# NVorbis/NVorbis

Measured on AMD Instinct MI355X. Metric: decoded Vorbis frames/sec (44.1 kHz stereo long-block), higher is better.
Workload: dtype f32; 1 GPU; C2: 4096 stereo long-block (n=2048) frames, Floor1+Residue2+coupling, IMDCT+window+OLA; frames_per_gpu=4096, channels=2, block=2048, parallelism=frame-parallel x1, 3 HIP streams per GPU x 3 resident batches each

## Files before the change

include/nvorbis_hip.h:

```cpp
#ifndef NVORBIS_HIP_H
#define NVORBIS_HIP_H

#include <stddef.h>
#include <stdint.h>

#ifdef __cplusplus
extern "C" {
#endif

#define NVH_OK 0
#define NVH_ERR_INVALID_DATA (-1)
#define NVH_ERR_ARGUMENT (-2)
#define NVH_ERR_RUNTIME (-3)
#define NVH_ERR_NOMEM (-4)
#define NVH_ERR_NOT_VORBIS (-5)
#define NVH_ERR_DEVICE (-6)
#define NVH_ERR_UNSUPPORTED (-7)
#define NVH_ERR_NO_GPU (-8)

typedef struct nvh_ctx nvh_ctx;
typedef struct nvh_stream nvh_stream;
typedef struct nvh_batch nvh_batch;

#define NVH_PKT_EOS 1
// ... 46 lines not shown
int nvh_mdct_reverse(nvh_ctx *ctx, int n, int batch, float *d_buf, int64_t stride);

int nvh_mdct_tables(int n, float *a , float *b , float *c , uint16_t *bitrev );
int nvh_calc_window(int prev_block, int block, int next_block, float *out );
int nvh_calc_overlap(int prev_block, int block, int next_block, int *start, int *valid, int *total);


int nvh_stream_open(nvh_ctx *ctx, const uint8_t *id_pkt, int id_len, const uint8_t *comment_pkt, int comment_len,
                    const uint8_t *setup_pkt, int setup_len, nvh_stream **out);
void nvh_stream_close(nvh_stream *s);
int nvh_stream_bitrates(const nvh_stream *s, int *upper, int *nominal, int *lower);
int nvh_stream_info(const nvh_stream *s, int *channels, int *sample_rate, int *block0, int *block1);
int nvh_pinned_alloc(size_t bytes, void **out);
void nvh_pinned_free(void *p);
int nvh_stream_set_clip(nvh_stream *s, int on);
int nvh_stream_set_gpu_parse(nvh_stream *s, int on);
int nvh_stream_has_clipped(nvh_stream *s, int *clipped);
int nvh_stream_position(const nvh_stream *s, int64_t *position, int64_t *emitted, int *eos);

int nvh_stream_push_packet(nvh_stream *s, const uint8_t *data, int len, int64_t granule, int flags);
int nvh_stream_push_packets(nvh_stream *s, const uint8_t *bytes, const int64_t *offsets, const int64_t *granules,
                            const uint8_t *flags, int n, int max_packets, int *consumed);
int nvh_stream_position_state(const nvh_stream *s, int *has_position, int64_t *position);
int nvh_stream_set_position_state(nvh_stream *s, int has_position, int64_t position);
int nvh_stream_index_packets(const nvh_stream *s, const uint8_t *bytes, const int64_t *offsets, const int64_t *granules,
                             const uint8_t *flags, int n, int64_t *position_after, int64_t *emitted_after,
                             uint8_t *state_after, int64_t *total_emitted);
int nvh_stream_packet_sample_count(const nvh_stream *s, const uint8_t *pkt, int len, int is_resync, int *count);
int nvh_stream_reset(nvh_stream *s);
int nvh_stream_drop_pending(nvh_stream *s);
int nvh_stream_push_end(nvh_stream *s);
int nvh_stream_pending_geometry(const nvh_stream *s, int32_t *out, int cap_frames);
int nvh_stream_pending(const nvh_stream *s, int *frames, int64_t *pcm_samples_per_channel);
int nvh_stream_next_segment(nvh_stream *s, int align);
int nvh_stream_segment_window(nvh_stream *s, int64_t skip, int64_t take, int64_t pitch);
int nvh_stream_pending_segments(const nvh_stream *s, int64_t *index, int64_t *begin, int64_t *end, int cap, int *count);
int nvh_stream_synth_segments(const nvh_stream *s, int64_t *index, int64_t *begin, int64_t *end, int cap, int *count);
int nvh_stream_synth_segments_clipped(const nvh_stream *s, int32_t *clipped, int cap, int *count);
int nvh_stream_pending_slabs(const nvh_stream *s, uint8_t *buf, int64_t cap, int64_t *bytes, uint32_t *first_unit,
                             int cap_frames);
int nvh_stream_lattice_pool(const nvh_stream *s, uint32_t *out, int64_t cap_words, int64_t *words);
int nvh_stream_vq_pool(const nvh_stream *s, float *out, int64_t cap_floats, int64_t *floats);

typedef struct nvh_pcm_out {
  int32_t format;
  int32_t mix;
  int32_t planar;
  int32_t out_channels;
  const int32_t *map;
  int64_t extent;
} nvh_pcm_out;
int nvh_stream_synth_out(nvh_stream *s, const nvh_pcm_out *out, void *pcm_host, void *d_pcm, int64_t *written);
int nvh_stream_synth_begin_out(nvh_stream *s, const nvh_pcm_out *out, void *pcm_host, int64_t *expected);

int nvh_stream_synth(nvh_stream *s, float *pcm_host, float *d_pcm, int64_t capacity, int64_t *written);
int nvh_stream_synth_begin(nvh_stream *s, float *pcm_host, int64_t capacity, int64_t *expected);
int nvh_stream_synth_end(nvh_stream *s, int64_t *written);
#define NVH_PCM_F32 0
#define NVH_PCM_S16 1
int nvh_stream_synth_pcm(nvh_stream *s, int format, void *pcm_host, void *d_pcm, int64_t capacity, int64_t *written);
int nvh_stream_synth_begin_pcm(nvh_stream *s, int format, void *pcm_host, int64_t capacity, int64_t *expected);
int nvh_stream_synth_planar(nvh_stream *s, int format, void *pcm_host, void *d_pcm, int64_t plane_stride, int64_t *written);
int nvh_stream_synth_begin_planar(nvh_stream *s, int format, void *pcm_host, int64_t plane_stride, int64_t *expected);
#define NVH_MIX_NONE 0
#define NVH_MIX_MONO 1
int nvh_stream_synth_mix(nvh_stream *s, int format, int mix, void *pcm_host, void *d_pcm, int64_t capacity, int64_t *written);
int nvh_stream_synth_begin_mix(nvh_stream *s, int format, int mix, void *pcm_host, int64_t capacity, int64_t *expected);
int nvh_channel_map_wave(int channels, int32_t *map);
int nvh_stream_synth_map(nvh_stream *s, int format, const int32_t *map, int out_channels, void *pcm_host, void *d_pcm, int64_t capacity, int64_t *written);
int nvh_stream_synth_begin_map(nvh_stream *s, int format, const int32_t *map, int out_channels, void *pcm_host, int64_t capacity, int64_t *expected);
int nvh_stream_synth_planar_map(nvh_stream *s, int format, const int32_t *map, int out_channels, void *pcm_host, void *d_pcm, int64_t plane_stride, int64_t *written);
int nvh_stream_synth_begin_planar_map(nvh_stream *s, int format, const int32_t *map, int out_channels, void *pcm_host, int64_t plane_stride, int64_t *expected);
int nvh_stream_parse_errors(const nvh_stream *s, int32_t *codes, int64_t *samples_before, int cap, int *count);

int nvh_mode_decode(nvh_stream *s, const uint8_t *pkt, int len, float *d_block, int *decoded, int *block_size, int *start,
                    int *valid, int *total);

int nvh_batch_upload(nvh_stream *s, nvh_batch **out);
int nvh_batch_info(const nvh_batch *b, int *frames, int *chan_frames, int64_t *pcm_samples_per_channel,
                   int64_t *descriptor_bytes);
int nvh_batch_stats(const nvh_batch *b, int64_t *out8);
int nvh_batch_kernels(const nvh_batch *b, char *buf, int cap);
int nvh_stream_kernels(const nvh_stream *s, char *buf, int cap);
int nvh_batch_synth_out(nvh_batch *b, const nvh_pcm_out *out, void *d_pcm);
int nvh_batch_synth(nvh_batch *b, float *d_pcm, int64_t capacity);
int nvh_batch_synth_pcm(nvh_batch *b, int format, void *d_pcm, int64_t capacity);
int nvh_batch_synth_planar(nvh_batch *b, int format, void *d_pcm, int64_t plane_stride);
int nvh_batch_synth_mix(nvh_batch *b, int format, int mix, void *d_pcm, int64_t capacity);
int nvh_batch_synth_map(nvh_batch *b, int format, const int32_t *map, int out_channels, void *d_pcm, int64_t capacity);
int nvh_batch_synth_planar_map(nvh_batch *b, int format, const int32_t *map, int out_channels, void *d_pcm, int64_t plane_stride);
int nvh_batch_time(nvh_batch *b, float *d_pcm, int64_t capacity, int iters, float *total_ms, float *kernel_ms );
void nvh_batch_free(nvh_batch *b);

int nvh_ogg_demux(const uint8_t *bytes, size_t len, uint8_t *pkt_bytes, int64_t pkt_bytes_cap, int64_t *offsets,
                  int64_t *granules, uint8_t *flags, int pkt_cap, int *npackets, int64_t *total_bytes);
int nvh_ogg_demux_stream(const uint8_t *bytes, size_t len, int stream_index, uint8_t *pkt_bytes, int64_t pkt_bytes_cap,
                         int64_t *offsets, int64_t *granules, uint8_t *flags, int pkt_cap, int *npackets,
                         int64_t *total_bytes, int *nstreams);

int nvh_ogg_index_packets(const uint8_t *bytes, size_t len, int stream_index, uint8_t *pkt_bytes, int64_t pkt_bytes_cap,
                          int64_t *offsets, int64_t *granules, uint8_t *flags, int pkt_cap, int *npackets,
                          int64_t *total_bytes, int64_t *payload_bytes, int *nstreams);

int nvh_ogg_demux_forward(const uint8_t *bytes, size_t len, int stream_index, uint8_t *pkt_bytes, int64_t pkt_bytes_cap,
                          int64_t *offsets, int64_t *granules, uint8_t *flags, int pkt_cap, int *npackets,
                          int64_t *total_bytes, int *nstreams);

typedef struct nvh_ogg_index nvh_ogg_index;
int nvh_ogg_index_open(const uint8_t *bytes, size_t len, int stream_index, nvh_ogg_index **out);
void nvh_ogg_index_close(nvh_ogg_index *ix);
int nvh_ogg_index_info(const nvh_ogg_index *ix, int *npages, int *npackets, int *first_data_page, int64_t *max_granule,
                       int *has_all_pages);
int nvh_ogg_index_page(const nvh_ogg_index *ix, int page, int64_t *granule, int *flags, int *packet_count, int *first_packet);
int nvh_ogg_seek(const nvh_ogg_index *ix, const nvh_stream *s, int64_t granule_pos, int pre_roll, int64_t *packet_index,
                 int64_t *granule_out);

#define NVH_RESAMPLE_TILE 512
typedef struct nvh_resample_desc {
  int32_t in_rate, out_rate;
  int32_t rows;
  int32_t channels;
  int32_t format;
  int32_t reserved;
  int64_t length;
  int64_t src_length;
  int64_t src_row_stride, src_time_stride, src_chan_stride;
  int64_t dst_row_stride, dst_time_stride, dst_chan_stride;
} nvh_resample_desc;
int nvh_resample_plan(int in_rate, int out_rate, int *up, int *down, int *half, int64_t *tap_count);
int nvh_resample_taps(int in_rate, int out_rate, float *taps, int64_t cap, int64_t *count);
int nvh_resample_rows(nvh_ctx *ctx, const nvh_resample_desc *desc, const float *d_src, void *d_dst, const int64_t *origin,
                      const int64_t *start, const int64_t *valid, const int32_t *dst_row, int32_t *d_clipped);
int nvh_resample_route(const nvh_resample_desc *desc, int64_t *out);

#define NVH_MEL_HTK 0
#define NVH_MEL_SLANEY 1
#define NVH_MEL_NORM_NONE 0
#define NVH_MEL_NORM_SLANEY 1
#define NVH_MEL_POWER 0
#define NVH_MEL_LN 1
#define NVH_MEL_DB 2
#define NVH_MEL_FRAMES 4
typedef struct nvh_mel_desc {
  int32_t rate, n_fft, win_length, hop, n_mels;
  int32_t mel_scale, norm, scale;
  float floor;
  int32_t rows;
  int32_t channels;
  int32_t reserved;
  double f_min, f_max;
  int64_t frames;
  int64_t first;
  int64_t src_length;
  int64_t src_row_stride, src_time_stride, src_chan_stride;
  int64_t dst_row_stride, dst_chan_stride, dst_frame_stride, dst_band_stride;
} nvh_mel_desc;
int nvh_mel_plan(const nvh_mel_desc *desc, int64_t *twiddle_count, int64_t *window_count, int64_t *bank_count);
int nvh_mel_tables(const nvh_mel_desc *desc, float *twiddle, float *window, float *bank, int64_t twiddle_cap, int64_t window_cap,
                   int64_t bank_cap, int64_t *twiddle_count, int64_t *window_count, int64_t *bank_count);
int nvh_mel_rows(nvh_ctx *ctx, const nvh_mel_desc *desc, const float *d_src, float *d_dst, const int64_t *valid);

#define NVH_WIN_HANN 0
#define NVH_WIN_HANN_SYM 1
#define NVH_WIN_HAMMING 2
#define NVH_WIN_POVEY 3
#define NVH_WIN_RECT 4
// ... 88 lines not shown
```

nvorbis_amd/csrc/kernels_synth.hip:

```cpp
#include <hip/hip_runtime.h>

#include "imdct_wave.h"
#include "kernels_common.h"
#include "spectrum_dev.h"

#include <type_traits>

namespace {

#ifdef NVH_NO_SYNTH_PF
constexpr bool kSynthPF = false, kSynthPFEmit = false;
#else
constexpr bool kSynthPF = true, kSynthPFEmit = true;
#endif
#ifdef NVH_ABL_NO_XFORM
constexpr int kAblSkip = 3;
#else
constexpr int kAblSkip = 0;
#endif

template <int AUX = 0>
__device__ __forceinline__ void dma16(const uint4* __restrict__ gsrc, float* lds_chunk_base) {
  __builtin_amdgcn_global_load_lds((const __attribute__((address_space(1))) void*)gsrc,
                                   (__attribute__((address_space(3))) void*)lds_chunk_base, 16, 0, AUX);
// ... 160 lines not shown
        if (!mg1) {
#pragma unroll
          for (int m = 0; m < G / 2; ++m) couple1(a[2 * m], a[2 * m + 1]);
        } else {
#pragma unroll
          for (int m = 0; m < G / 2; ++m) couple1(a[2 * m + 1], a[2 * m]);
        }
      }
      float* p0 = spec + xb;
      float* p1 = spec + (unsigned)half + xb;
      if constexpr (FUSE && G == 8) {
        if (xb + 4 <= (unsigned)half) {
#pragma unroll
          for (int c = 0; c < 2; ++c) {
            if (F->md[c] == 1) {
              float m[4];
              floor_walk_fx<4>(F->seg[c], F->tab[c], F->s_db, (int)xb, m);
#pragma unroll
              for (int q = 0; q < 4; ++q) a[2 * q + c] = a[2 * q + c] * m[q];
            } else if (F->md[c] == 2) {
#pragma unroll
              for (int q = 0; q < 4; ++q) a[2 * q + c] = 0.0f;
            }
          }
          *reinterpret_cast<float4*>(p0) = make_float4(a[0], a[2], a[4 % G], a[6 % G]);
          *reinterpret_cast<float4*>(p1) = make_float4(a[1], a[3 % G], a[5 % G], a[7 % G]);
        }
      } else
      if (G == 8 && (xb & 3u) == 0 && xb + 4 <= (unsigned)half) {
        *reinterpret_cast<float4*>(p0) = make_float4(a[0], a[2], a[4 % G], a[6 % G]);
        *reinterpret_cast<float4*>(p1) = make_float4(a[1], a[3 % G], a[5 % G], a[7 % G]);
      } else {
#pragma unroll
        for (int m = 0; m < G / 2; ++m)
          if (xb + m < (unsigned)half) {
            p0[m] = a[2 * m];
            p1[m] = a[2 * m + 1];
          }
      }
    } else {
      const unsigned c = (rec.y >> 25) & 7u;
      const unsigned xb = xbase + i0;
      float* p = spec + c * (unsigned)half + xb;
      if constexpr (FUSE && G == 8) {
        if (xb + 8 <= (unsigned)half) {
          const bool c1 = c != 0;
          const int md = c1 ? F->md[1] : F->md[0];
          if (md == 1) {
            float m[8];
            floor_walk_fx<8>(c1 ? F->seg[1] : F->seg[0], c1 ? F->tab[1] : F->tab[0], F->s_db, (int)xb, m);
#pragma unroll
            for (int q = 0; q < 8; ++q) a[q % G] = a[q % G] * m[q];
          } else if (md == 2) {
#pragma unroll
            for (int q = 0; q < G; ++q) a[q] = 0.0f;
          }
          *reinterpret_cast<float4*>(p) = make_float4(a[0], a[1], a[2 % G], a[3 % G]);
          *reinterpret_cast<float4*>(p + 4) = make_float4(a[4 % G], a[5 % G], a[6 % G], a[7 % G]);
        } else if (xb + 4 <= (unsigned)half) {
          __builtin_trap();
        }
      } else
      if (G == 8 && (xb & 3u) == 0 && xb + 8 <= (unsigned)half) {
        *reinterpret_cast<float4*>(p) = make_float4(a[0], a[1], a[2 % G], a[3 % G]);
        *reinterpret_cast<float4*>(p + 4) = make_float4(a[4 % G], a[5 % G], a[6 % G], a[7 % G]);
      } else {
#pragma unroll
        for (int k = 0; k < G; ++k)
          if (xb + k < (unsigned)half) p[k] = a[k];
      }
    }
  }
}


struct WalkFrame {
  const float* slab;
  unsigned off_heads, off_rec, off_ent, nheads, lpc, lpc_magic, flags;
  float* spec;
  int half;
  FloorRef F;
};

template <int NT>
__device__ __forceinline__ void residue_walk_two(const WalkFrame (&W)[2], const uint32_t* __restrict__ s_lat, int tid) {
  constexpr int G = 8;
  const uint32_t* heads[2];
  const uint2* recs[2];
  const uint8_t* ent[2];
  unsigned total[2];
#pragma unroll
  for (int f = 0; f < 2; ++f) {
    heads[f] = reinterpret_cast<const uint32_t*>(W[f].slab + W[f].off_heads * 4);
    recs[f] = reinterpret_cast<const uint2*>(W[f].slab + W[f].off_rec * 4);
    ent[f] = reinterpret_cast<const uint8_t*>(W[f].slab + W[f].off_ent * 4);
    total[f] = W[f].nheads * W[f].lpc;
  }
  const unsigned tmax = total[0] > total[1] ? total[0] : total[1];
  for (unsigned idx = tid; idx < tmax; idx += NT) {
    bool act[2], more[2];
    unsigned o[2], xbase[2], i0[2];
    uint2 rec[2];
    float a[2][G];
#pragma unroll
    for (int f = 0; f < 2; ++f) {
      act[f] = idx < total[f];
      const unsigned ii = act[f] ? idx : 0u;
      const unsigned oq = W[f].lpc > 1 ? __umulhi(ii, W[f].lpc_magic) : ii;
      i0[f] = (ii - oq * W[f].lpc) * G;
      const unsigned hd = heads[f][oq];
      o[f] = hd & 0xFFFFu;
      xbase[f] = hd >> 16;
      rec[f] = recs[f][o[f]];
      more[f] = act[f];
#pragma unroll
      for (int k = 0; k < G; ++k) a[f][k] = 0.0f;
    }
#ifdef NVH_ABL_NO_CHAIN2
    more[0] = more[1] = false;
#endif
    while (more[0] | more[1]) {
      float v[2][G];
#pragma unroll
      for (int f = 0; f < 2; ++f) {
        const char* vb = reinterpret_cast<const char*>(s_lat) + ((rec[f].y & 0xFFFu) << 2);
        const uint8_t* db = ent[f] + ((rec[f].x & 0xFFFFu) << 1) + i0[f];
        const uint2 w = *reinterpret_cast<const uint2*>(db);
#pragma unroll
        for (int k = 0; k < 4; ++k) {
          v[f][k] = *reinterpret_cast<const float*>(vb + ((w.x >> (8 * k)) & 0xFFu));
          v[f][4 + k] = *reinterpret_cast<const float*>(vb + ((w.y >> (8 * k)) & 0xFFu));
        }
      }
#pragma unroll
      for (int f = 0; f < 2; ++f) {
        const uint32_t keep = more[f] ? 0xFFFFFFFFu : 0u;
#pragma unroll
        for (int k = 0; k < G; ++k) a[f][k] = a[f][k] + __uint_as_float(__float_as_uint(v[f][k]) & keep);
        more[f] = more[f] && (rec[f].y & 0x80000000u) != 0u;
        o[f] += more[f] ? 1u : 0u;
        rec[f] = recs[f][o[f]];
      }
    }
#pragma unroll
    for (int f = 0; f < 2; ++f) {
      if (!act[f]) continue;
      const unsigned xb = xbase[f] + (i0[f] >> 1);
      if (W[f].flags & NVH_SLAB_SWEEP_COUPLES) {
        if (!(W[f].flags & NVH_SLAB_MG1)) {
#pragma unroll
          for (int m = 0; m < G / 2; ++m) couple1(a[f][2 * m], a[f][2 * m + 1]);
        } else {
#pragma unroll
          for (int m = 0; m < G / 2; ++m) couple1(a[f][2 * m + 1], a[f][2 * m]);
        }
      }
      if (xb + 4 <= (unsigned)W[f].half) {
#pragma unroll
        for (int c = 0; c < 2; ++c) {
#ifdef NVH_ABL_NO_FLOOR2
          if (false) {
#else
          if (W[f].F.md[c] == 1) {
#endif
            float m[4];
            floor_walk_fx<4>(W[f].F.seg[c], W[f].F.tab[c], W[f].F.s_db, (int)xb, m);
#pragma unroll
            for (int q = 0; q < 4; ++q) a[f][2 * q + c] = a[f][2 * q + c] * m[q];
          } else if (W[f].F.md[c] == 2) {
#pragma unroll
            for (int q = 0; q < 4; ++q) a[f][2 * q + c] = 0.0f;
          }
        }
        *reinterpret_cast<float4*>(W[f].spec + xb) = make_float4(a[f][0], a[f][2], a[f][4], a[f][6]);
        *reinterpret_cast<float4*>(W[f].spec + (unsigned)W[f].half + xb) = make_float4(a[f][1], a[f][3], a[f][5], a[f][7]);
      }
    }
  }
}

template <int NT, bool DIG = false>
__device__ __forceinline__ void residue_walk_bins(const float* slab, unsigned off_heads, unsigned off_rec, unsigned off_ent,
                                                  unsigned off_bins, unsigned psz_magic, const uint32_t* __restrict__ s_lat,
                                                  float* spec, int half, unsigned rch, int tid, const float* __restrict__ vq = nullptr) {
  const uint32_t* heads = reinterpret_cast<const uint32_t*>(slab + off_heads * 4);
  const uint2* recs = reinterpret_cast<const uint2*>(slab + off_rec * 4);
  const uint16_t* ent = reinterpret_cast<const uint16_t*>(slab + off_ent * 4);
  const uint32_t* prm = reinterpret_cast<const uint32_t*>(slab + off_bins * 4);
  const unsigned rbegin = __builtin_amdgcn_readfirstlane(prm[0]), psz = __builtin_amdgcn_readfirstlane(prm[1]);
  const unsigned nparts = __builtin_amdgcn_readfirstlane(prm[2]), cover = __builtin_amdgcn_readfirstlane(prm[3]);
  const uint16_t* pchain = reinterpret_cast<const uint16_t*>(prm + 4);
  if (nparts == 0) return;
  const unsigned rch_magic = (unsigned)((0x100000000ull + rch - 1) / rch);
  auto base_of = [&](unsigned p) { return __umulhi(rbegin + p * psz, rch_magic); };
  const unsigned xfirst = base_of(0), xend = base_of(nparts - 1) + cover;
  for (unsigned X = xfirst + (unsigned)tid; X < xend; X += NT) {
    unsigned phi = __umulhi((X + 1) * rch - 1 - rbegin, psz_magic);
    if (phi >= nparts) phi = nparts - 1;
    unsigned cb = pchain[phi], ca = 0xFFFFu;
    if (X >= base_of(phi) + cover) cb = 0xFFFFu;
    if (phi >= 1 && X < base_of(phi - 1) + cover) ca = pchain[phi - 1];
    unsigned oa = 0, ob = 0, xa = 0, xbb = 0;
    uint2 ra = make_uint2(0u, 0u), rb = ra;
    bool va = ca != 0xFFFFu, vb = cb != 0xFFFFu;
    if (va) { const unsigned hd = heads[ca]; oa = hd & 0xFFFFu; xa = hd >> 16; ra = recs[oa]; }
    if (vb) { const unsigned hd = heads[cb]; ob = hd & 0xFFFFu; xbb = hd >> 16; rb = recs[ob]; }
    float a[NVH_SLAB_MAX_CH];
#pragma unroll
    for (int c = 0; c < NVH_SLAB_MAX_CH; ++c) a[c] = 0.0f;
    while (va || vb) {
      const bool take_a = va && (!vb || ((ra.y >> 28) & 7u) <= ((rb.y >> 28) & 7u));
      const uint2 rec = take_a ? ra : rb;
      const unsigned q0 = (X - (take_a ? xa : xbb)) * rch;
      if constexpr (DIG) {
        const char* vb = reinterpret_cast<const char*>(s_lat) + ((rec.y & 0xFFFu) << 2);
        const uint8_t* db = reinterpret_cast<const uint8_t*>(ent) + ((rec.x & 0xFFFFu) << 1);
#pragma unroll
        for (int c = 0; c < NVH_SLAB_MAX_CH; ++c) {
          if ((unsigned)c < rch) {
            const unsigned q = q0 + (unsigned)c;
            const bool in = q < psz;
            const float v = *reinterpret_cast<const float*>(vb + db[in ? q : 0u]);
            a[c] = a[c] + (in ? v : 0.0f);
          }
        }
      } else {
      const unsigned dims = (rec.y >> 20) & 31u, lv = (rec.y >> 12) & 0xFFu, dm16 = rec.x >> 16;
      const uint32_t* lat = s_lat + (rec.y & 0xFFFu);
      const uint16_t* eb = ent + (rec.x & 0xFFFFu);
      const unsigned lvm = lat[lv + 1];
#pragma unroll
      for (int c = 0; c < NVH_SLAB_MAX_CH; ++c) {
        if ((unsigned)c < rch) {
          const unsigned q = q0 + (unsigned)c;
          const bool in = q < psz;
          const unsigned qq = in ? q : 0u;
          const unsigned j = (qq * dm16) >> 16, comp = qq - j * dims;
          const unsigned e = eb[j];
          float v;
          if (lv == 0u) {
            v = table_value(vq, lat, dims, e, comp);
          } else {
            const unsigned pw = lat[lv + comp];
            const unsigned qv = comp ? __umulhi(e, pw) : e;
            const unsigned dgt = qv - __umul24(__umulhi(qv, lvm), lv);
            v = __uint_as_float(lat[dgt]);
// ... 961 lines not shown
  } else {
    bool kept = false;
    if constexpr (MAXCH > 2 && MODE >= 2) kept = xform && direct8;
    if constexpr (MAXCH > 2 && MODE >= 2) if (kept) {
      const float* X = spec + wv * half;
      float* scratch = smem + wv * (half + (n >> 4));
      switch (n) {
        case 256: imdct_keep_quarters<8>(X, scratch, Aa, Bb, Cc, TW, lane); break;
        case 512: imdct_keep_quarters<9>(X, scratch, Aa, Bb, Cc, TW, lane); break;
        case 1024: imdct_keep_quarters<10>(X, scratch, Aa, Bb, Cc, TW, lane); break;
        case 2048: imdct_keep_quarters<11>(X, scratch, Aa, Bb, Cc, TW, lane); break;
        case 4096: imdct_keep_quarters<12>(X, scratch, Aa, Bb, Cc, TW, lane); break;
        default: __builtin_trap();
      }
    }
    if (xform && !kept) {
      const float* X = spec + wv * half;
      float* out = planes + (long long)wv * A.block1;
      float* scratch = smem + wv * (half + (n >> 4));
      switch (n) {
        case 256: imdct_wave<8, false, true, true, true, false, true>(X, out, nullptr, scratch, Aa, Bb, Cc, TW, lane); break;
        case 512: imdct_wave<9, false, true, true, true, false, true>(X, out, nullptr, scratch, Aa, Bb, Cc, TW, lane); break;
        case 1024: imdct_wave<10, false, true, true, true, false, true>(X, out, nullptr, scratch, Aa, Bb, Cc, TW, lane); break;
        case 2048: imdct_wave<11, false, true, true, true, false, true>(X, out, nullptr, scratch, Aa, Bb, Cc, TW, lane); break;
        case 4096: imdct_wave<12, false, true, true, true, false, true>(X, out, nullptr, scratch, Aa, Bb, Cc, TW, lane); break;
        case 8192: {
          __syncthreads();
          float* own = spec + nch * half_max + wv * (half + (n >> 4));
          imdct_wave<13, false, true>(X, out, nullptr, own, Aa, Bb, Cc, TW, lane);
          break;
        }
        default: __builtin_trap();
      }
    }
  }
  if (!xform && wv < nch) {
    const float* X = spec + wv * half;
    float* out = planes + (long long)wv * A.block1;
    for (int i = lane * 4; i < half; i += 256) *reinterpret_cast<float4*>(out + i) = *reinterpret_cast<const float4*>(X + i);
    for (int i = lane * 4; i < (half >> 1); i += 256) *reinterpret_cast<float4*>(out + half + i) = make_float4(0.0f, 0.0f, 0.0f, 0.0f);
  }
  if (MAXCH > 2 && !xform) __syncthreads();
  if constexpr (MAXCH > 2 && MODE >= 2) {
    const unsigned ef = ef8;
    if (direct8) {
      __syncthreads();
      switch (nch) {
        case 1: synth_emit8_direct<NT, 1, PCM, LAYOUT>(A, smem, n, frame, tid, cm); break;
        case 2: synth_emit8_direct<NT, 2, PCM, LAYOUT>(A, smem, n, frame, tid, cm); break;
        case 3: synth_emit8_direct<NT, 3, PCM, LAYOUT>(A, smem, n, frame, tid, cm); break;
        case 4: synth_emit8_direct<NT, 4, PCM, LAYOUT>(A, smem, n, frame, tid, cm); break;
        case 5: synth_emit8_direct<NT, 5, PCM, LAYOUT>(A, smem, n, frame, tid, cm); break;
        case 6: synth_emit8_direct<NT, 6, PCM, LAYOUT>(A, smem, n, frame, tid, cm); break;
        case 7: synth_emit8_direct<NT, 7, PCM, LAYOUT>(A, smem, n, frame, tid, cm); break;
        case 8: synth_emit8_direct<NT, 8, PCM, LAYOUT>(A, smem, n, frame, tid, cm); break;
        default: __builtin_trap();
      }
    } else
    if (ef & (NVH_EMIT_SELF | NVH_EMIT_NEXT | NVH_EMIT_CARRY_OUT)) {
      __syncthreads();
      if ((ef & NVH_EMIT_CARRY_OUT) && A.carry_out) synth_carry_out8<NT>(A, planes, n, nch, exec_mask, A.frames[frame].window_off, tid);
      if (ef & (NVH_EMIT_SELF | NVH_EMIT_NEXT)) synth_emit8<NT, PCM, LAYOUT>(A, smem, n, nch, frame, ef, exec_mask, tid, cm);
    }
  }
  if constexpr (MAXCH > 2 && MODE < 2) {
    if (A.carry_out != nullptr && (A.frames[frame].emit_flags & NVH_EMIT_CARRY_OUT)) {
      __syncthreads();
      synth_carry_out8<NT>(A, planes, n, nch, exec_mask, A.frames[frame].window_off, tid);
    }
  }
  if constexpr (MAXCH <= 2 && MODE >= 1) {
    if (carry_out && !(emit_self || emit_next)) {
      __syncthreads();
      synth_carry_out<NT>(A, planes, n, nch, exec_mask, carry_window, tid);
    }
  }
  SY_T(5);
#ifdef NVH_DEBUG
  if (dbg && threadIdx.x == 0) dbg[(long long)f * 24 + 23] = wall_clock64();
#endif
#undef SY_T
}

template <int NT, int FPW, typename PCM = float, int LAYOUT = NVH_LAYOUT_INTERLEAVED>
__device__ __forceinline__ void synth_group_body(const NvhSynthArgs& A, float* smem NVH_DBG_PARAMS) {
  static_assert(NT / 64 >= 2 * FPW, "one wavefront per (frame, channel) in the transform");
  constexpr bool PLANAR = LAYOUT == NVH_LAYOUT_PLANAR, MONO = LAYOUT == NVH_LAYOUT_MONO;
  const int tid = threadIdx.x, wv = __builtin_amdgcn_readfirstlane(tid >> 6), lane = tid & 63;
  const int nch = A.channels;
  const int fa = A.f0 + (int)blockIdx.x * A.fstep;
#ifdef NVH_DEBUG
#define GR_T(k) do { if (dbg && tid == 0 && fa < A.nframes) dbg[(long long)fa * 24 + (k)] = clock64(); } while (0)
#else
#define GR_T(k) do { } while (0)
#endif
  GR_T(0);
  const int half_max = A.block1 >> 1, pad_max = A.block1 >> 4;
  float* s_db = smem;
  const uint32_t* s_lat = reinterpret_cast<const uint32_t*>(smem + 256);
  float* slab0 = smem + A.const_vecs * 4;
  const int slab_words = A.lds_vecs * 4;
  float* spec0 = slab0 + FPW * slab_words;
  const int region = nch * half_max;
  const int slice_words = half_max + pad_max;
  float* slice0 = smem + nch * half_max;
  const int walk_end = A.const_vecs * 4 + FPW * (slab_words + region), xform_end = nch * half_max + FPW * nch * slice_words;
  uint32_t* otab = reinterpret_cast<uint32_t*>(smem + (walk_end > xform_end ? walk_end : xform_end));
  typedef const __attribute__((address_space(4))) uint32_t* const_words;
  unsigned w0[FPW], w3[FPW];
#pragma unroll
  for (int k = 0; k < FPW; ++k) {
    w0[k] = 0u; w3[k] = 0u;
    if (fa + k < A.nframes) {
      const uint4* gslab = A.slabs + (long long)(fa + k) * A.stride_vecs;
      const_words gh = (const_words)(unsigned long long)gslab;
      w0[k] = gh[0]; w3[k] = gh[3];
      if (tid < A.cap_vecs) dma16<kSlabAux>(gslab + tid, slab0 + k * slab_words + wv * 256);
    }
  }
  for (int c0 = wv * 64; c0 < A.const_vecs; c0 += NT)
    if (c0 + lane < A.const_vecs) dma16(A.consts + c0 + lane, smem + c0 * 4);
  {
    const float4 z = make_float4(0.0f, 0.0f, 0.0f, 0.0f);
#pragma unroll
    for (int k = 0; k < FPW; ++k) {
      float4* sp = reinterpret_cast<float4*>(spec0 + k * region);
      for (int i = tid; i < (nch * half_max) >> 2; i += NT) sp[i] = z;
    }
  }
  int nn[FPW];
  bool any = false;
#pragma unroll
  for (int k = 0; k < FPW; ++k) {
    nn[k] = (int)(w0[k] & 0xFFFFu);
    any = any || nn[k] != 0;
    const unsigned vecs = w3[k] >> 16;
    if ((int)vecs > A.cap_vecs) __builtin_trap();
    if (vecs > (unsigned)NT) {
      const uint4* gslab = A.slabs + (long long)(fa + k) * A.stride_vecs;
      for (unsigned c0 = NT + wv * 64; c0 < vecs; c0 += NT)
        if (c0 + lane < vecs) dma16<kSlabAux>(gslab + c0 + lane, slab0 + k * slab_words + c0 * 4);
    }
  }
  if (A.prefetch_prev && wv == NT / 64 - 1 && fa >= FPW) {
    const int lines = (A.cap_vecs < 256 ? A.cap_vecs : 256) >> 3;
#pragma unroll
    for (int k = 0; k < FPW; ++k)
      if (lane < lines) {
        const volatile unsigned* pp = reinterpret_cast<const volatile unsigned*>(A.slabs + (long long)(fa - FPW + k) * A.stride_vecs) + lane * 32;
        (void)*pp;
      }
  }
  __syncthreads();
  if (!any) return;
  GR_T(1);

  auto hdr = [&](int k, int i) { return __builtin_amdgcn_readfirstlane(reinterpret_cast<const uint32_t*>(slab0 + k * slab_words)[i]); };
  {
    bool together = false;
    if constexpr (FPW == 2) {
      WalkFrame W[2];
      together = A.walk_two != 0;
#pragma unroll
      for (int k = 0; k < 2; ++k) {
        const unsigned w1 = hdr(k, 1), w2 = hdr(k, 2), w4 = hdr(k, 4), flags = w0[k] >> 24, rgeom = (w4 >> 16) & 0xFFu;
        W[k].slab = slab0 + k * slab_words;
        W[k].nheads = w1 & 0xFFFFu; W[k].off_heads = w2 & 0xFFFFu; W[k].off_rec = w2 >> 16; W[k].off_ent = w3[k] & 0xFFFFu;
        W[k].lpc = w4 & 0xFFFFu; W[k].lpc_magic = hdr(k, 5); W[k].flags = flags;
        W[k].spec = spec0 + k * region; W[k].half = nn[k] >> 1;
        together = together && nn[k] != 0 && (flags & NVH_SLAB_FUSE_FLOOR) && !(flags & NVH_SLAB_FLOOR_FAULT) &&
                   rgeom == (2u | NVH_SLAB_RGEOM_DIGITS | (2u << 4)) && (w4 >> 24) == 8u && W[k].nheads * W[k].lpc != 0u;
        const uint32_t* s_chan = reinterpret_cast<const uint32_t*>(W[k].slab) + 8;
        const unsigned c0w = __builtin_amdgcn_readfirstlane(s_chan[0]), c1w = __builtin_amdgcn_readfirstlane(s_chan[1]);
        const unsigned cw[2] = {c0w, c1w};
#pragma unroll
        for (int c = 0; c < 2; ++c) {
          const unsigned ns = (cw[c] >> 8) & 0xFFu, oseg = cw[c] >> 16;
          W[k].F.seg[c] = reinterpret_cast<const uint4*>(W[k].slab + oseg * 4);
          W[k].F.tab[c] = reinterpret_cast<const uint8_t*>(W[k].slab + (oseg + ns) * 4);
          W[k].F.md[c] = (int)(cw[c] & 0xFFu);
        }
        W[k].F.s_db = s_db;
      }
      if (together) residue_walk_two<NT>(W, s_lat, tid);
      if (together) { GR_T(2); GR_T(3); }
    }
    if (!together)
#pragma unroll
    for (int k = 0; k < FPW; ++k) {
      if (nn[k] != 0)
        synth_frame_spectrum<NT, 2, false>(A, s_db, s_lat, slab0 + k * slab_words, spec0 + k * region, w0[k], hdr(k, 1), hdr(k, 2),
                                           w3[k], hdr(k, 4), hdr(k, 5), hdr(k, 7), tid);
      if (k < 2) GR_T(2 + k);
    }
  }

  const bool emit = A.pcm != nullptr;
  bool self_k[FPW], next_k[FPW], cout_k[FPW], done_k[FPW];
  bool self_carry = false;
  int gprev[FPW], gnext[FPW], gstart[FPW], gvalid[FPW];
#pragma unroll
  for (int k = 0; k < FPW; ++k) {
    const unsigned flags = w0[k] >> 24, xm = (w0[k] >> 16) & 0xFFu;
    self_k[k] = emit && nn[k] != 0 && (flags & NVH_SLAB_EMIT_SELF);
    next_k[k] = emit && nn[k] != 0 && (flags & NVH_SLAB_EMIT_NEXT);
    done_k[k] = emit && nn[k] != 0 && (xm & NVH_SLABX_DONE);
    cout_k[k] = A.carry_out != nullptr && nn[k] != 0 && (xm & NVH_SLABX_CARRY_OUT);
    if (k == 0) self_carry = self_k[0] && (xm & NVH_SLABX_SELF_CARRY);
    const unsigned geo = (self_k[k] || next_k[k] || done_k[k]) ? hdr(k, 13) : 0u;
    gprev[k] = (int)(geo & 0xFFu) << 6; gnext[k] = (int)((geo >> 8) & 0xFFu) << 6;
    gstart[k] = (int)((geo >> 16) & 0xFFu) << 6; gvalid[k] = (int)(geo >> 24) << 6;
  }
  bool act[FPW + 1];
  act[0] = self_k[0] && !self_carry;
#pragma unroll
  for (int j = 1; j < FPW; ++j) act[j] = next_k[j - 1] && self_k[j] && nn[j] == gnext[j - 1];
  act[FPW] = next_k[FPW - 1];
  int mov[FPW + 1];
  mov[0] = nn[0] < gprev[0] ? nn[0] : gprev[0];
#pragma unroll
  for (int j = 1; j <= FPW; ++j) mov[j] = nn[j - 1] < gnext[j - 1] ? nn[j - 1] : gnext[j - 1];
  int r1len[FPW], r2len[FPW];
#pragma unroll
  for (int k = 0; k < FPW; ++k) {
    const int mk = nn[k] < gprev[k] ? nn[k] : gprev[k];
    r1len[k] = done_k[k] ? (nn[k] >> 1) - gstart[k] - (mk >> 1) : 0;
    r2len[k] = done_k[k] ? gvalid[k] - (nn[k] >> 1) : 0;
    if (r1len[k] < 0 || r2len[k] < 0 || r1len[k] > (nn[k] >> 2) || r2len[k] > (nn[k] >> 2)) __builtin_trap();
  }
  const int S0 = (int)(slice0 - smem), SK = nch * slice_words;
  if (tid <= FPW) {
    const int j = tid, kb = j == 0 ? 0 : j - 1;
    const uint32_t* H = reinterpret_cast<const uint32_t*>(slab0 + kb * slab_words);
    const int n = (int)(H[0] & 0xFFFFu);
    const unsigned geo = H[13];
    uint4 r0, r1;
    if (j == 0) {
      const int pn = (int)(geo & 0xFFu) << 6, m = n < pn ? n : pn, start = (int)((geo >> 16) & 0xFFu) << 6;
// ... 51 lines not shown
    bool wrA = true, wrB = true, keep = false;
#pragma unroll
    for (int kk = 0; kk < FPW; ++kk)
      if (kk == k) {
        n = nn[kk]; mw0 = w0[kk];
        const bool a_here = kk == 0 ? self_k[0] : act[kk], b_here = kk == FPW - 1 ? next_k[FPW - 1] : act[kk + 1];
        wrA = !a_here || cout_k[kk] || !done_k[kk];
        wrB = !b_here || cout_k[kk] || !done_k[kk];
        keep = a_here || b_here || done_k[kk];
      }
    const unsigned exec_mask = (mw0 >> 16) & 0xFFu, flags = mw0 >> 24;
    const int half = n >> 1;
    const int sl = (flags & NVH_SLAB_MDCT_SLOT) ? 1 : 0;
    const float* X = spec0 + k * region + c * half;
    float* slice = slice0 + (k * nch + c) * slice_words;
    float* plane = A.work + ((long long)(fa + k) * nch + c) * A.block1;
    const bool mine = tw && c < nch && n != 0;
    if (mine && !((exec_mask >> c) & 1u)) {
      for (int i = lane * 4; i < half; i += 256) *reinterpret_cast<float4*>(plane + i) = *reinterpret_cast<const float4*>(X + i);
      for (int i = lane * 4; i < (half >> 1); i += 256) *reinterpret_cast<float4*>(plane + half + i) = make_float4(0.0f, 0.0f, 0.0f, 0.0f);
    }
    if (mine && ((exec_mask >> c) & 1u)) {
      float4 ca[2] = {make_float4(0.f, 0.f, 0.f, 0.f), make_float4(0.f, 0.f, 0.f, 0.f)}, cb[2] = {ca[0], ca[0]};
      auto sink = [&](int slot, int, float4 v) {
        if (slot == 0) ca[0] = v; else if (slot == 2) cb[0] = v; else if (slot == 4) ca[1] = v; else if (slot == 6) cb[1] = v;
      };
      const float* Aa = A.mdct_a[sl];
      const float* Bb = A.mdct_b[sl];
      const float* Cc = A.mdct_c[sl];
      const float* TW = A.mdct_tw[sl];
      switch (n) {
        case 256: imdct_wave_sink<8, false, decltype(sink), true, true, false, kSynthPFEmit, true>(X, nullptr, slice, Aa, Bb, Cc, TW, lane, sink, nullptr, kAblSkip); break;
        case 512: imdct_wave_sink<9, false, decltype(sink), true, true, false, kSynthPFEmit, true>(X, nullptr, slice, Aa, Bb, Cc, TW, lane, sink, nullptr, kAblSkip); break;
        case 1024: imdct_wave_sink<10, false, decltype(sink), true, true, false, kSynthPFEmit, true>(X, nullptr, slice, Aa, Bb, Cc, TW, lane, sink, nullptr, kAblSkip); break;
        case 2048: imdct_wave_sink<11, false, decltype(sink), true, true, false, kSynthPFEmit, true>(X, nullptr, slice, Aa, Bb, Cc, TW, lane, sink, nullptr, kAblSkip); break;
        default: __builtin_trap();
      }
      if (lane < (n >> 5)) {
        const int i8a = lane, i8b = (n >> 4) - 1 - lane;
        if (wrA) {
          *reinterpret_cast<float4*>(plane + 4 * i8a) = ca[0];
          *reinterpret_cast<float4*>(plane + 4 * i8b) = ca[1];
        }
        if (wrB) {
          *reinterpret_cast<float4*>(plane + half + 4 * i8a) = cb[0];
          *reinterpret_cast<float4*>(plane + half + 4 * i8b) = cb[1];
        }
        if (keep) {
          float* own = slice;
          *reinterpret_cast<float4*>(own + 4 * i8a) = ca[0];
          *reinterpret_cast<float4*>(own + 4 * i8b) = ca[1];
          *reinterpret_cast<float4*>(own + (half >> 1) + 4 * i8a) = cb[0];
          *reinterpret_cast<float4*>(own + (half >> 1) + 4 * i8b) = cb[1];
        }
      }
    } else {
      lds_barrier();
    }
  }
  GR_T(5);
  __syncthreads();
  GR_T(6);

#pragma unroll
  for (int k = 0; k < FPW; ++k)
    if (cout_k[k])
      synth_carry_out<NT>(A, A.work + (long long)(fa + k) * nch * A.block1, nn[k], nch, (w0[k] >> 16) & 0xFFu, cwin[k], tid);
  if (self_carry)
    synth_self_carry<NT, PCM, LAYOUT>(A, slice0, nn[0], nch, __builtin_amdgcn_readfirstlane(otab[0]), __builtin_amdgcn_readfirstlane(otab[2]), tid, fa, slice_words);

  int cnt[FPW + 2];
  cnt[0] = 0;
#pragma unroll
  for (int j = 0; j <= FPW; ++j) cnt[j + 1] = cnt[j] + (act[j] ? (mov[j] >> 4) : 0);
  int clipped = 0;
  for (int t = tid; t < cnt[FPW + 1]; t += NT) {
    int j = 0;
#pragma unroll
    for (int jj = 1; jj <= FPW; ++jj) j += (int)(t >= cnt[jj]);
    int g = t;
#pragma unroll
    for (int jj = 1; jj <= FPW; ++jj) g = j == jj ? t - cnt[jj] : g;
    const uint4 r0 = reinterpret_cast<const uint4*>(otab)[2 * j], r1 = reinterpret_cast<const uint4*>(otab)[2 * j + 1];
    const int n = (int)r0.w, half = n >> 1, i0 = 4 * g;
    const int cbit = 1 << j;
    const float* __restrict__ w = A.windows + r0.x;
    const float* __restrict__ wp = A.windows + r0.y;
    const float4 wf = *reinterpret_cast<const float4*>(w + i0);
    const float4 wm = *reinterpret_cast<const float4*>(w + (half - 4 - i0));
    const float4 pf = *reinterpret_cast<const float4*>(wp + i0);
    const float4 pm = *reinterpret_cast<const float4*>(wp + (half - 4 - i0));
    float fwd[8], mir[8];
#pragma unroll
    for (int c = 0; c < 2; ++c) {
      if (c < nch) {
        const float4 a = *reinterpret_cast<const float4*>(smem + r1.x + c * r1.y + i0);
        const float4 b = *reinterpret_cast<const float4*>(smem + r1.z + c * r1.w + i0);
        float4 v = make_float4(a.x * wf.x, a.y * wf.y, a.z * wf.z, a.w * wf.w);
        const float4 tt = make_float4(b.x * pf.x, b.y * pf.y, b.z * pf.z, b.w * pf.w);
        v.x = v.x + tt.x; v.y = v.y + tt.y; v.z = v.z + tt.z; v.w = v.w + tt.w;
        float4 u = make_float4(-a.w * wm.x, -a.z * wm.y, -a.y * wm.z, -a.x * wm.w);
        const float4 r = make_float4(b.w * pm.x, b.z * pm.y, b.y * pm.z, b.x * pm.w);
        u.x = u.x + r.x; u.y = u.y + r.y; u.z = u.z + r.z; u.w = u.w + r.w;
        if (!MONO && A.clip) {
          v.x = clip_value(v.x, &clipped, cbit); v.y = clip_value(v.y, &clipped, cbit);
          v.z = clip_value(v.z, &clipped, cbit); v.w = clip_value(v.w, &clipped, cbit);
          u.x = clip_value(u.x, &clipped, cbit); u.y = clip_value(u.y, &clipped, cbit);
          u.z = clip_value(u.z, &clipped, cbit); u.w = clip_value(u.w, &clipped, cbit);
        }
        if constexpr (PLANAR) {
          pcm_store_plane(reinterpret_cast<PCM*>(A.pcm) + (long long)r0.z + (long long)c * A.plane_stride, g, (n >> 3) - 1 - g, v, u);
        } else {
          fwd[c] = v.x; fwd[2 + c] = v.y; fwd[4 + c] = v.z; fwd[6 + c] = v.w;
            mir[c] = u.x; mir[2 + c] = u.y; mir[4 + c] = u.z; mir[6 + c] = u.w;
        }
      }
    }
    PCM* out = reinterpret_cast<PCM*>(A.pcm) + (long long)r0.z * (PLANAR || MONO ? 1 : nch);
    if constexpr (PLANAR) {
    } else if constexpr (MONO) {
      pcm_store_plane(out, g, (n >> 3) - 1 - g, mono_mix2(fwd, nch, A.clip, &clipped, cbit), mono_mix2(mir, nch, A.clip, &clipped, cbit));
    } else if (nch == 2) {
      pcm4_t<PCM>* of = reinterpret_cast<pcm4_t<PCM>*>(out) + 2 * (long long)g;
      pcm4_t<PCM>* om = reinterpret_cast<pcm4_t<PCM>*>(out) + 2 * (long long)((n >> 3) - 1 - g);
      if constexpr (std::is_same<PCM, int16_t>::value) {
        pcm_store4x2(of, fwd);
        pcm_store4x2(om, mir);
      } else {
        pcm_store4(of, fwd[0], fwd[1], fwd[2], fwd[3]);
        pcm_store4(of + 1, fwd[4], fwd[5], fwd[6], fwd[7]);
        pcm_store4(om, mir[0], mir[1], mir[2], mir[3]);
        pcm_store4(om + 1, mir[4], mir[5], mir[6], mir[7]);
      }
    } else {
      pcm_store4(reinterpret_cast<pcm4_t<PCM>*>(out) + g, fwd[0], fwd[2], fwd[4], fwd[6]);
      pcm_store4(reinterpret_cast<pcm4_t<PCM>*>(out) + ((n >> 3) - 1 - g), mir[0], mir[2], mir[4], mir[6]);
    }
  }
  int fcnt[FPW + 1];
  fcnt[0] = 0;
#pragma unroll
  for (int k = 0; k < FPW; ++k) fcnt[k + 1] = fcnt[k] + ((r1len[k] + r2len[k]) >> 2);
  for (int t = tid; t < fcnt[FPW]; t += NT) {
    int k = 0;
#pragma unroll
    for (int kk = 1; kk < FPW; ++kk) k += (int)(t >= fcnt[kk]);
    int g = t;
#pragma unroll
    for (int kk = 1; kk < FPW; ++kk) g = k == kk ? t - fcnt[kk] : g;
    const uint4 r0 = reinterpret_cast<const uint4*>(otab)[2 * (FPW + 1 + k)], r1 = reinterpret_cast<const uint4*>(otab)[2 * (FPW + 1 + k) + 1];
    const int n = (int)r0.z, q1 = (int)(r1.y >> 2);
    const bool second = g >= q1;
    const int cbit = 1 << k;
    const int idx0 = second ? (n >> 1) + 4 * (g - q1) : (int)r1.x + 4 * g;
    const float4 wv4 = *reinterpret_cast<const float4*>(A.windows + r0.x + idx0);
    const int src = second ? (n >> 2) + (idx0 - (n >> 1)) : (n >> 1) - 4 - idx0;
    float o[8];
#pragma unroll
    for (int c = 0; c < 2; ++c) {
      if (c < nch) {
        const float4 x = *reinterpret_cast<const float4*>(smem + r0.w + c * slice_words + src);
        float4 v = second ? make_float4(x.x * wv4.x, x.y * wv4.y, x.z * wv4.z, x.w * wv4.w)
                          : make_float4(-x.w * wv4.x, -x.z * wv4.y, -x.y * wv4.z, -x.x * wv4.w);
        if (!MONO && A.clip) {
          v.x = clip_value(v.x, &clipped, cbit); v.y = clip_value(v.y, &clipped, cbit);
          v.z = clip_value(v.z, &clipped, cbit); v.w = clip_value(v.w, &clipped, cbit);
        }
        if constexpr (PLANAR)
          pcm_store4(reinterpret_cast<pcm4_t<PCM>*>(reinterpret_cast<PCM*>(A.pcm) + ((long long)r0.y + (idx0 - (int)r1.w)) +
                                                    (long long)c * A.plane_stride), v.x, v.y, v.z, v.w);
        else {
          o[c] = v.x; o[2 + c] = v.y; o[4 + c] = v.z; o[6 + c] = v.w;
        }
      }
    }
    PCM* out = reinterpret_cast<PCM*>(A.pcm) + ((long long)r0.y + (idx0 - (int)r1.w)) * (PLANAR || MONO ? 1 : nch);
    if constexpr (PLANAR) {
    } else if constexpr (MONO) {
      const float4 m = mono_mix2(o, nch, A.clip, &clipped, cbit);
      pcm_store4(reinterpret_cast<pcm4_t<PCM>*>(out), m.x, m.y, m.z, m.w);
    } else if (nch == 2) {
      if constexpr (std::is_same<PCM, int16_t>::value) {
        pcm_store4x2(reinterpret_cast<pcm4_t<PCM>*>(out), o);
      } else {
        pcm_store4(reinterpret_cast<float4*>(out), o[0], o[1], o[2], o[3]);
        pcm_store4(reinterpret_cast<float4*>(out) + 1, o[4], o[5], o[6], o[7]);
      }
    } else {
      pcm_store4(reinterpret_cast<pcm4_t<PCM>*>(out), o[0], o[2], o[4], o[6]);
    }
  }
  if (A.clip && emit) report_clipped<FPW + 1>(clipped, A.clipped_flag, fa);
  GR_T(7);
#undef GR_T
}

#ifndef NVH_SYNTH_NT
#define NVH_SYNTH_NT SP_THREADS
#define NVH_SYNTH_WPE 8, 8
#endif
extern "C" __global__ void __launch_bounds__(NVH_SYNTH_NT) __attribute__((amdgpu_waves_per_eu(NVH_SYNTH_WPE)))
k_synth(NvhSynthArgs A NVH_DBG_PARAMS) {
  extern __shared__ __attribute__((aligned(16))) float smem[];
  synth_body<NVH_SYNTH_NT, 2>(A, smem NVH_DBG_ARGS);
}

extern "C" __global__ void __launch_bounds__(NVH_SYNTH_NT) __attribute__((amdgpu_waves_per_eu(NVH_SYNTH_WPE)))
k_synth_tail(NvhSynthArgs A NVH_DBG_PARAMS) {
  extern __shared__ __attribute__((aligned(16))) float smem[];
  synth_body<NVH_SYNTH_NT, 2, 1>(A, smem NVH_DBG_ARGS);
}

#define NVH_SYNTH_EMIT(PCM, LAYOUT, SFX)                                                                                   \
  extern "C" __global__ void __launch_bounds__(NVH_SYNTH_NT) __attribute__((amdgpu_waves_per_eu(NVH_SYNTH_WPE)))           \
  k_synth_emit##SFX(NvhSynthArgs A NVH_DBG_PARAMS) {                                                                       \
    extern __shared__ __attribute__((aligned(16))) float smem[];                                                           \
    synth_body<NVH_SYNTH_NT, 2, 2, false, PCM, LAYOUT>(A, smem NVH_DBG_ARGS);                                              \
  }
NVH_FOR_PCM_TWINS(NVH_SYNTH_EMIT)

// ... 46 lines not shown
```

nvorbis_amd/csrc/nvh_api.hip:

```cpp
#include "nvh_internal.h"

#include <bitset>

thread_local int g_last_hip_error = 0;

const NvhToggles& nvh_toggles() {
  static const NvhToggles t = [] {
    auto on = [](const char* k) { return std::getenv(k) != nullptr; };
    auto num = [](const char* k) { const char* v = std::getenv(k); return v ? std::atoi(v) : 0; };
    NvhToggles x{};
    x.no_compact = on("NVH_NO_COMPACT");
    x.no_fused_imdct = on("NVH_NO_FUSED_IMDCT");
    x.no_gen8 = on("NVH_NO_GEN8");
    x.unfused = on("NVH_UNFUSED");
    x.no_pair = on("NVH_NO_PAIR");
    x.no_slab = on("NVH_NO_SLAB");
    x.uncached_planes = on("NVH_UNCACHED_PLANES");
    x.poison_planes = on("NVH_POISON_PLANES");
    x.no_ola_sym = on("NVH_NO_OLA_SYM");
    x.no_emit = on("NVH_NO_EMIT");
    x.emit8 = on("NVH_EMIT8");
    x.no_emit8 = on("NVH_NO_EMIT8");
    x.no_prefetch = on("NVH_NO_PREFETCH");
    x.no_walk_two = on("NVH_NO_WALK_TWO");
    x.fpw = std::getenv("NVH_FPW") ? num("NVH_FPW") : 2;
    if (x.fpw != 1 && x.fpw != 2 && x.fpw != 4) x.fpw = 2;
    x.copy_upload = on("NVH_COPY_UPLOAD");
    x.xcd_map = on("NVH_XCD_MAP");
    x.emit_always = on("NVH_EMIT_ALWAYS");
    x.debug_occ = on("NVH_DEBUG_OCC");
    x.gpu_parse_default = on("NVH_GPU_PARSE");
    x.lds_pad = num("NVH_LDS_PAD");
    x.ola_threads = num("NVH_OLA_THREADS");
    x.parse_lanes = num("NVH_PARSE_LANES");
    x.parse_waves = num("NVH_PARSE_WAVES");
    x.no_parse_uni = on("NVH_NO_PARSE_UNI");
    x.no_parse_sub = on("NVH_NO_PARSE_SUB");
    x.parse_cur = std::getenv("NVH_PARSE_CUR") ? num("NVH_PARSE_CUR") : -1;
    if (x.parse_cur > 2) x.parse_cur = 2;
    x.no_sleep_wait = on("NVH_NO_SLEEP_WAIT");
    x.no_parse_sort = on("NVH_NO_PARSE_SORT");
    x.ola_segs = num("NVH_OLA_SEGS");
    x.zero_chunk_kib = num("NVH_ZERO_CHUNK_KIB");
    x.phase_mask = std::getenv("NVH_DEBUG_SPECTRUM_MASK") ? num("NVH_DEBUG_SPECTRUM_MASK") : 15;
    return x;
  }();
  return t;
}

#ifdef NVH_DEBUG
void* g_dbg_buf = nullptr;
extern "C" void nvh_debug_set_buffer(void* d_buf) { g_dbg_buf = d_buf; }
#endif

static int ensure_device(int device) {
  int count = 0;
  hipError_t e = hipGetDeviceCount(&count);
  if (e != hipSuccess || count <= 0) {
    g_last_hip_error = (int)e;
    return NVH_ERR_NO_GPU;
  }
  if (device < 0 || device >= count) return NVH_ERR_ARGUMENT;
  HIP_TRY(hipSetDevice(device));
  return NVH_OK;
}

#ifndef NVH_SRC_HASH
#define NVH_SRC_HASH "unknown"
#endif
extern "C" const char* nvh_version(void) { return "nvorbis_hip 0.3 (gfx950) nvh-src-hash=" NVH_SRC_HASH; }
extern "C" int nvh_last_hip_error(void) { return g_last_hip_error; }
extern "C" int nvh_device_count(void) {
  int count = 0;
  if (hipGetDeviceCount(&count) != hipSuccess) return 0;
  return count;
}

extern "C" int nvh_ctx_create(int device, nvh_ctx** out) {
  return nvh_guard([&]() -> int {
    if (!out) return NVH_ERR_ARGUMENT;
    *out = nullptr;
    int rc = ensure_device(device);
    if (rc != NVH_OK) return rc;
    nvh_ctx* c = new (std::nothrow) nvh_ctx();
    if (!c) return NVH_ERR_NOMEM;
    c->device = device;
    c->hpool.host = true;
    hipError_t e = hipStreamCreateWithFlags(&c->stream, hipStreamNonBlocking);
    if (e != hipSuccess) {
      g_last_hip_error = (int)e;
      delete c;
      return NVH_ERR_DEVICE;
    }
    c->own_stream = true;
    *out = c;
    return NVH_OK;
  });
}

extern "C" void nvh_ctx_destroy(nvh_ctx* c) {
  nvh_guard_void([&] {
    if (!c) return;
    (void)hipSetDevice(c->device);
    for (auto& kv : c->mdct_cache) kv.second.free_tables();
    for (auto& kv : c->resample_cache) (void)hipFree(kv.second.taps);
    c->resample_rows.release();
    for (auto& kv : c->mel_cache) kv.second.free_tables();
// ... 830 lines not shown
    return F.replay_error;
  });
}

extern "C" int nvh_stream_parse_errors(const nvh_stream* s, int32_t* codes, int64_t* samples_before, int cap, int* count) {
  return nvh_guard([&]() -> int {
    if (!s || !count || cap < 0 || (cap > 0 && (!codes || !samples_before))) return NVH_ERR_ARGUMENT;
    const int n = s->replay_error != NVH_OK ? (int)s->replay_errors.size() : 0;
    *count = n;
    for (int i = 0; i < n && i < cap; i++) {
      codes[i] = s->replay_errors[(size_t)i].first;
      samples_before[i] = s->replay_errors[(size_t)i].second;
    }
    return NVH_OK;
  });
}

extern "C" int nvh_batch_upload(nvh_stream* s, nvh_batch** out) {
  return nvh_guard([&]() -> int {
    if (!s || !out) return NVH_ERR_ARGUMENT;
    *out = nullptr;
    if (!s->ctx) return NVH_ERR_NO_GPU;
    HIP_TRY(hipSetDevice(s->ctx->device));
    std::unique_ptr<nvh_batch> b(new (std::nothrow) nvh_batch());
    if (b && s && s->ctx) {
      b->blob.pool = b->work.pool = b->carry_in.pool = b->slabs.pool = b->dev_copy.pool = b->slab3.pool = b->gap_dev.pool = &s->ctx->pool;
      b->work.uncached = nvh_toggles().uncached_planes;
      b->h_blob.host = b->gap_host.host = true;
      b->h_blob.pool = b->gap_host.pool = &s->ctx->hpool;
    }
    if (!b) return NVH_ERR_NOMEM;
    size_t plane = (size_t)s->setup.channels * (size_t)s->setup.block1 * sizeof(float);
    int rc = b->carry_in.reserve(plane);
    if (rc != NVH_OK) return rc;
    HIP_TRY(hipMemcpyAsync(b->carry_in.p, s->carry[s->carry_cur].p, plane, hipMemcpyDeviceToDevice, s->ctx->stream));
    b->has_carry_in = true;
    s->replay_error = NVH_OK;
    rc = batch_upload(s, b.get());
    if (rc != NVH_OK) return rc;
    if (s->replay_error != NVH_OK) return s->replay_error;
    *out = b.release();
    return NVH_OK;
  });
}

extern "C" int nvh_batch_info(const nvh_batch* b, int* frames, int* chan_frames, int64_t* pcm_samples,
                              int64_t* descriptor_bytes) {
  return nvh_guard([&]() -> int {
    if (!b) return NVH_ERR_ARGUMENT;
    if (frames) *frames = b->nframes;
    if (chan_frames) *chan_frames = b->chan_frames;
    if (pcm_samples) *pcm_samples = b->pcm_samples;
    if (descriptor_bytes) *descriptor_bytes = b->descriptor_bytes;
    return NVH_OK;
  });
}

extern "C" int nvh_batch_stats(const nvh_batch* b, int64_t* out8) {
  return nvh_guard([&]() -> int {
    if (!b || !out8) return NVH_ERR_ARGUMENT;
    for (int i = 0; i < 8; i++) out8[i] = b->stats[i];
    return NVH_OK;
  });
}

extern "C" int nvh_batch_kernels(const nvh_batch* b, char* buf, int cap) {
  return nvh_guard([&]() -> int {
    if (!b || !buf || cap <= 0) return NVH_ERR_ARGUMENT;
    std::string t;
    for (int k = 0; k < 4; k++) {
      if (k) t += ",";
      t += b->slot_name[k];
    }
    if ((int)t.size() + 1 > cap) return NVH_ERR_ARGUMENT;
    std::memcpy(buf, t.c_str(), t.size() + 1);
    return NVH_OK;
  });
}

extern "C" int nvh_stream_kernels(const nvh_stream* s, char* buf, int cap) {
  return nvh_batch_kernels(s ? &s->scratch : nullptr, buf, cap);
}

static int batch_out(nvh_batch* b, const nvh_pcm_out* d, void* d_pcm, NamedForm form = kDescriptor) {
  return nvh_guard([&]() -> int {
    nvh_stream* s = b ? b->s : nullptr;
    PcmOut out;
    const int rc = resolve_out(s, b, d, form, false, nullptr, d_pcm, nullptr, &out);
    if (rc != NVH_OK) return rc;
    HIP_TRY(hipSetDevice(s->ctx->device));
    return batch_launch(b, (const float*)b->carry_in.p, (float*)s->carry[s->carry_cur].p, d_pcm, false, nullptr, nullptr, out);
  });
}

extern "C" int nvh_batch_synth_out(nvh_batch* b, const nvh_pcm_out* out, void* d_pcm) { return batch_out(b, out, d_pcm); }

extern "C" int nvh_batch_synth(nvh_batch* b, float* d_pcm, int64_t capacity) {
  const nvh_pcm_out d{NVH_PCM_F32, NVH_MIX_NONE, 0, 0, nullptr, capacity};
  return nvh_batch_synth_out(b, &d, d_pcm);
}

extern "C" int nvh_batch_synth_pcm(nvh_batch* b, int format, void* d_pcm, int64_t capacity) {
  const nvh_pcm_out d{format, NVH_MIX_NONE, 0, 0, nullptr, capacity};
  return nvh_batch_synth_out(b, &d, d_pcm);
}

extern "C" int nvh_batch_synth_mix(nvh_batch* b, int format, int mix, void* d_pcm, int64_t capacity) {
  const nvh_pcm_out d{format, mix, 0, 0, nullptr, capacity};
  return nvh_batch_synth_out(b, &d, d_pcm);
}

extern "C" int nvh_batch_synth_planar(nvh_batch* b, int format, void* d_pcm, int64_t plane_stride) {
  const nvh_pcm_out d{format, NVH_MIX_NONE, 1, 0, nullptr, plane_stride};
  return nvh_batch_synth_out(b, &d, d_pcm);
}

extern "C" int nvh_batch_synth_map(nvh_batch* b, int format, const int32_t* map, int out_channels, void* d_pcm, int64_t capacity) {
  const nvh_pcm_out d{format, NVH_MIX_NONE, 0, out_channels, map, capacity};
  return batch_out(b, &d, d_pcm, kNamedMap);
}

extern "C" int nvh_batch_synth_planar_map(nvh_batch* b, int format, const int32_t* map, int out_channels, void* d_pcm,
                                          int64_t plane_stride) {
  const nvh_pcm_out d{format, NVH_MIX_NONE, 1, out_channels, map, plane_stride};
  return batch_out(b, &d, d_pcm, kNamedMap);
}

extern "C" int nvh_batch_time(nvh_batch* b, float* d_pcm, int64_t capacity, int iters, float* total_ms,
                              float* kernel_ms) {
  return nvh_guard([&]() -> int {
    if (!b || !b->s || iters <= 0) return NVH_ERR_ARGUMENT;
    nvh_stream* s = b->s;
    if (capacity < b->pcm_samples * s->setup.channels) return NVH_ERR_ARGUMENT;
    HIP_TRY(hipSetDevice(s->ctx->device));
    hipStream_t st = s->ctx->stream;
    float km[4] = {0, 0, 0, 0};
    if (kernel_ms) {
      std::vector<ScopedEvent> evs((size_t)iters * 5);
      std::vector<hipEvent_t> raw((size_t)iters * 5);
      for (size_t k = 0; k < evs.size(); k++) {
        int rc = evs[k].create();
        if (rc != NVH_OK) return rc;
        raw[k] = evs[k].e;
      }
      for (int i = 0; i < iters; i++) {
        int rc = batch_launch(b, (const float*)b->carry_in.p, (float*)s->carry[s->carry_cur].p, d_pcm, true, km, &raw[(size_t)i * 5]);
        if (rc != NVH_OK) return rc;
      }
      HIP_TRY(hipEventSynchronize(raw.back()));
      for (int i = 0; i < iters; i++)
        for (int k = 0; k < 4; k++) {
          float ms = 0;
          HIP_TRY(hipEventElapsedTime(&ms, raw[(size_t)i * 5 + k], raw[(size_t)i * 5 + k + 1]));
          km[k] += ms;
        }
      for (int k = 0; k < 4; k++) kernel_ms[k] = km[k] / (float)iters;
    }
    if (total_ms) {
      ScopedEvent e0, e1;
      int rc = e0.create();
      if (rc == NVH_OK) rc = e1.create();
      if (rc != NVH_OK) return rc;
      HIP_TRY(hipEventRecord(e0.e, st));
      for (int i = 0; i < iters; i++) {
        rc = batch_launch(b, (const float*)b->carry_in.p, (float*)s->carry[s->carry_cur].p, d_pcm, false, nullptr);
        if (rc != NVH_OK) return rc;
// ... 220 lines not shown
```

nvorbis_amd/csrc/nvh_format.h:

```cpp
#pragma once
#include <stdint.h>

#define NVH_MAX_POSTS 64
#define NVH_LINK_NONE 0x7FFF
#define NVH_MAX_STAGES 8
#define NVH_MAX_CLASSES 64
#define NVH_ENTRY_SKIP 0xFFFFu


struct NvhDevBook {
  uint32_t tab_off;
  uint32_t entries;
  uint32_t dim;
  uint32_t dim_magic;
  uint32_t lat_values;
  uint32_t lat_magic;
  uint32_t lat_off;
  uint32_t dim_magic16;
};

struct NvhDevFloor1 {
  int32_t x_count;
  int32_t multiplier;
  int32_t range;
// ... 38 lines not shown
  int32_t pair_path;
  uint32_t hp_magic;
  int32_t alias_b1;
  int32_t pad[2];
};

struct NvhDevMapping {
  int32_t coupling_steps;
  uint32_t coupling_off;
};


struct NvhResOp {
  uint32_t ent_off;
  uint16_t partition;
  uint8_t channel;
  uint8_t book;
};

struct NvhResPass {
  int32_t residue;
  uint32_t op_begin[NVH_MAX_STAGES + 1];
};

struct NvhChan {
  uint8_t exec;
  uint8_t floor;
  uint8_t post_count;
  uint8_t ov_exec;
  uint32_t data_off;
  float amp;
};

struct NvhFrame {
  int32_t n;
  int32_t mapping;
  uint32_t window_off;
  int32_t mdct_slot;
  int32_t start, valid, total;
  int32_t emit_start;
  int32_t emit_count;
  int32_t ov_frame;
  int32_t ov_src;
  int32_t ov_len;
  int64_t out_pos;
  uint32_t chan_off;
  uint32_t pass_begin, pass_end;
  uint32_t op_begin, op_count;
  uint32_t ent_begin, ent_count;
  int32_t ov_n;
  uint32_t ov_window_off;
  uint32_t exec_mask;
  uint32_t ov_exec_mask;
  uint32_t emit_flags;
};

#define NVH_EMIT_SELF 1u
#define NVH_EMIT_NEXT 2u
#define NVH_EMIT_DONE 4u
#define NVH_EMIT_SELF_CARRY 8u
#define NVH_EMIT_CARRY_OUT 16u

#define NVH_SLAB_REC(ent_off, dm16, lat_off, lat_values, dim, channel, stage, more)                                              \
  ((uint32_t)(ent_off) | ((uint32_t)(dm16) << 16)),                                                                               \
      ((uint32_t)(lat_off) | ((uint32_t)(lat_values) << 12) | ((uint32_t)(dim) << 20) | ((uint32_t)(channel) << 25) |             \
       ((uint32_t)(stage) << 28) | ((more) ? 0x80000000u : 0u))
#define NVH_SLAB_MAX_LAT_OFF 0xFFFu
#define NVH_SLAB_RGEOM_DIGITS 8u
#define NVH_SLAB_MAX_DIGIT 63u
#define NVH_SLAB_SWEEP_COUPLES 1u
#define NVH_SLAB_MG1 2u
#define NVH_SLAB_COUPLE_PASS 4u
#define NVH_SLAB_FLOOR_FAULT 8u
#define NVH_SLAB_MDCT_SLOT 16u
#define NVH_SLAB_FUSE_FLOOR 32u
#define NVH_SLAB_EMIT_SELF 64u
#define NVH_SLAB_EMIT_NEXT 128u
#define NVH_SLABX_SELF_CARRY 0x40u
#define NVH_SLABX_CARRY_OUT 0x80u
#define NVH_SLABX_DONE 0x20u
#define NVH_SLAB_GEO(prev_n, next_n, start, valid) \
  ((uint32_t)((prev_n) >> 6) | ((uint32_t)((next_n) >> 6) << 8) | ((uint32_t)((start) >> 6) << 16) | ((uint32_t)((valid) >> 6) << 24))
#define NVH_SLAB_HDR_VECS 4
#define NVH_SLAB_MAX_CH 8
#define NVH_SLAB_MAX_COUPLE 4
struct NvhSlabHdr {
  uint16_t n;
  uint8_t exec_mask;
  uint8_t flags;
  uint16_t nheads, nrec;
  uint16_t off_heads, off_rec;
  uint16_t off_ent;
  uint16_t vecs;
  uint16_t lpc;
  uint8_t rgeom;
  uint8_t group;
  uint32_t lpc_magic;
  uint32_t frame;
  uint32_t coupling;
  uint32_t chan[NVH_SLAB_MAX_CH];
};
```

nvorbis_amd/csrc/nvh_internal.h:

```cpp
#pragma once
#include <time.h>
#include <hip/hip_runtime.h>

#include <algorithm>
#include <cstdio>
#include <cstdlib>
#include <cstring>
#include <initializer_list>
#include <iterator>
#include <map>
#include <memory>
#include <new>
#include <string>
#include <tuple>
#include <vector>

#include "../../include/nvorbis_hip.h"
#include "host_ogg.h"
#include "host_parse.h"
#include "host_setup.h"
#include "host_slab.h"
#include "kernels_common.h"
#include "nvh_parse_format.h"
#include "cep_dev.h"
// ... 67 lines not shown

template <typename PCM, int LAYOUT>
__global__ void k_ola_compact(NvhDevSetup S, NvhDevBatch Bt, const float* work, const float* carry, PCM* pcm, int clip,
                              int* clipped_flag, float* carry_out, int last_decoded, int nosym, const int* list, int emitted,
                              pcm_stride_t<LAYOUT> plane_stride);
template <typename PCM, int LAYOUT>
__global__ void k_ola_emit(NvhDevSetup S, NvhDevBatch Bt, const float* work, const float* carry, PCM* pcm, int clip, int* clipped_flag,
                           pcm_stride_t<LAYOUT> plane_stride);
template <typename PCM, int LAYOUT>
__global__ void k_ola_emit_seq(NvhDevSetup S, NvhDevBatch Bt, float* work, const float* carry, PCM* pcm, int clip, int* clipped_flag,
                               pcm_stride_t<LAYOUT> plane_stride);
#define NVH_OLA_DECL(PCM, LAYOUT, SFX)                                                                                               \
  extern template __global__ void k_ola_compact<PCM, LAYOUT>(NvhDevSetup, NvhDevBatch, const float*, const float*, PCM*, int, int*,  \
                                                             float*, int, int, const int*, int, pcm_stride_t<LAYOUT>);               \
  extern template __global__ void k_ola_emit<PCM, LAYOUT>(NvhDevSetup, NvhDevBatch, const float*, const float*, PCM*, int, int*,     \
                                                          pcm_stride_t<LAYOUT>);                                                     \
  extern template __global__ void k_ola_emit_seq<PCM, LAYOUT>(NvhDevSetup, NvhDevBatch, float*, const float*, PCM*, int, int*,       \
                                                              pcm_stride_t<LAYOUT>);
NVH_FOR_PCM_TWINS(NVH_OLA_DECL)
NVH_FOR_PCM_MAP_TWINS(NVH_OLA_DECL)

template <typename PCM>
__global__ void k_resample_rows(NvhResampleArgs A);
extern template __global__ void k_resample_rows<float>(NvhResampleArgs);
extern template __global__ void k_resample_rows<int16_t>(NvhResampleArgs);

template <bool STAGED, bool FRONT>
__global__ void k_mel_rows(NvhMelArgs A);
extern template __global__ void k_mel_rows<true, false>(NvhMelArgs);
extern template __global__ void k_mel_rows<false, false>(NvhMelArgs);
extern template __global__ void k_mel_rows<true, true>(NvhMelArgs);
extern template __global__ void k_mel_rows<false, true>(NvhMelArgs);

template <bool RESIDENT>
__global__ void k_fnorm_rows(NvhFnormArgs A);
extern template __global__ void k_fnorm_rows<true>(NvhFnormArgs);
extern template __global__ void k_fnorm_rows<false>(NvhFnormArgs);

template <bool STAGED>
__global__ void k_cep_rows(NvhCepArgs A);
extern template __global__ void k_cep_rows<true>(NvhCepArgs);
extern template __global__ void k_cep_rows<false>(NvhCepArgs);

extern thread_local int g_last_hip_error;

#define HIP_TRY(expr)                        \
  do {                                       \
    hipError_t e_ = (expr);                  \
    if (e_ != hipSuccess) {                  \
      g_last_hip_error = (int)e_;            \
      return NVH_ERR_DEVICE;                 \
    }                                        \
  } while (0)

template <class F>
static inline int nvh_guard(F&& body) noexcept {
  try {
    return body();
  } catch (const std::bad_alloc&) {
    return NVH_ERR_NOMEM;
  } catch (...) {
    return NVH_ERR_RUNTIME;
  }
}
template <class F>
static inline void nvh_guard_void(F&& body) noexcept {
  try {
    body();
  } catch (...) {
  }
}

struct NvhToggles {
  bool no_compact, no_fused_imdct, no_gen8, unfused, no_pair, debug_occ, gpu_parse_default;
  bool no_ola_sym;
  bool emit8;
  bool no_emit8;
  bool no_emit;
  bool emit_always;
  bool xcd_map;
  bool copy_upload;
  int fpw;
  bool no_walk_two;
  bool no_prefetch;
  bool uncached_planes;
  bool poison_planes;
  bool no_slab;
  int lds_pad, ola_threads, parse_lanes, parse_waves;
  bool no_sleep_wait;
  bool no_parse_sort;
  int parse_cur;
  bool no_parse_sub;
  bool no_parse_uni;
  int ola_segs;
  int zero_chunk_kib;
  int phase_mask;
};
const NvhToggles& nvh_toggles();
#ifdef NVH_DEBUG
extern void* g_dbg_buf;
#define NVH_DBG_LAUNCH , (long long*)g_dbg_buf, nvh_toggles().phase_mask
#else
#define NVH_DBG_LAUNCH
#endif

struct BufPool {
  bool host = false;
  std::multimap<size_t, void*> free_;
  size_t bytes_ = 0;
  void raw_free(void* p) const { (void)(host ? hipHostFree(p) : hipFree(p)); }
  static constexpr size_t kKeepBytes = (size_t)2 << 30;
  static size_t size_class(size_t bytes) {
    size_t v = bytes < 4096 ? 4096 : bytes;
    size_t p = 1;
    while ((p << 1) <= v) p <<= 1;
    size_t step = p >> 2;
    return (v + step - 1) / step * step;
  }
  void* take(size_t cls) {
    auto it = free_.find(cls);
    if (it == free_.end()) return nullptr;
    void* p = it->second;
    free_.erase(it);
    bytes_ -= cls;
    return p;
  }
  void give(void* p, size_t cls) {
    if (bytes_ + cls > kKeepBytes) {
      raw_free(p);
      return;
    }
    free_.emplace(cls, p);
    bytes_ += cls;
  }
  void clear() {
    for (auto& kv : free_) raw_free(kv.second);
    free_.clear();
    bytes_ = 0;
  }
};

struct DevBuf {
  void* p = nullptr;
  size_t cap = 0;
  BufPool* pool = nullptr;
  bool host = false;
  bool uncached = false;
  ~DevBuf() { release(); }
  void release() {
    if (!p) return;
    if (pool && !uncached) pool->give(p, cap);
    else (void)(host ? hipHostFree(p) : hipFree(p));
    p = nullptr;
    cap = 0;
  }
  int reserve(size_t bytes) {
    if (bytes <= cap) return NVH_OK;
    release();
    const size_t want = BufPool::size_class(bytes + 256);
    if (pool && !uncached) p = pool->take(want);
    if (!p) {
      if (host) HIP_TRY(hipHostMalloc(&p, want, hipHostMallocDefault));
      else if (uncached) HIP_TRY(hipExtMallocWithFlags(&p, want, hipDeviceMallocUncached));
      else HIP_TRY(hipMalloc(&p, want));
    }
    cap = want;
    return NVH_OK;
  }
};

template <class T>
static inline int upload_table(T** dst, const std::vector<T>& src) {
  void* p = nullptr;
  HIP_TRY(hipMalloc(&p, src.empty() ? 4 : src.size() * sizeof(T)));
  const hipError_t e = src.empty() ? hipSuccess : hipMemcpy(p, src.data(), src.size() * sizeof(T), hipMemcpyHostToDevice);
  if (e != hipSuccess) {
    (void)hipFree(p);
    g_last_hip_error = (int)e;
    return NVH_ERR_DEVICE;
  }
  *dst = static_cast<T*>(p);
// ... 67 lines not shown
  BufPool pool;
  BufPool hpool;
  std::map<std::string, std::shared_ptr<SharedSetup>> setup_cache;
  bool big_lds_attr_set = false;
  bool group_lds_attr_set = false;
  bool synth_lds_attr_set = false;
  bool parse_lds_attr_set = false;
  int parse_lanes = 0;
  std::map<std::pair<int, int>, ResampleDev> resample_cache;
  std::map<MelKey, MelDev> mel_cache;
  std::map<CepKey, CepDev> cep_cache;
  bool resample_lds_attr_set = false, mel_lds_attr_set = false, fnorm_lds_attr_set = false, cep_lds_attr_set = false;
  RowBlock resample_rows, mel_rows, fnorm_rows, cep_rows;
};

inline int RowBlock::begin(nvh_ctx* c, size_t bytes, void** image) {
  if (!copied) HIP_TRY(hipEventCreateWithFlags(&copied, hipEventDisableTiming));
  else HIP_TRY(hipEventSynchronize(copied));
  host.host = true;
  host.pool = &c->hpool;
  dev.pool = &c->pool;
  int rc = host.reserve(bytes);
  if (rc == NVH_OK) rc = dev.reserve(bytes);
  if (rc == NVH_OK) *image = host.p;
  return rc;
}

inline int RowBlock::send(nvh_ctx* c, size_t bytes, const void** d_block) {
  HIP_TRY(hipMemcpyAsync(dev.p, host.p, bytes, hipMemcpyHostToDevice, c->stream));
  HIP_TRY(hipEventRecord(copied, c->stream));
  *d_block = dev.p;
  return NVH_OK;
}

static inline int lds_opt_in(bool& done, int bytes, std::initializer_list<const void*> kernels) {
  if (done) return NVH_OK;
  for (const void* k : kernels) HIP_TRY(hipFuncSetAttribute(k, hipFuncAttributeMaxDynamicSharedMemorySize, bytes));
  done = true;
  return NVH_OK;
}

inline hipError_t nvh_wait_stream(const nvh_ctx* c, hipStream_t st) {
  if (!c || c->parse_lanes <= 0 || nvh_toggles().no_sleep_wait) return hipStreamSynchronize(st);
  for (;;) {
    const hipError_t e = hipStreamQuery(st);
    if (e != hipErrorNotReady) return e;
    struct timespec ts = {0, 50 * 1000};
    nanosleep(&ts, nullptr);
  }
}

struct nvh_batch {
  nvh_stream* s = nullptr;
  DevBuf blob;
  DevBuf h_blob;
  DevBuf slabs;
  DevBuf work;
  DevBuf carry_in;
  NvhDevBatch dev{};
  int nframes = 0, chan_frames = 0;
  int64_t pcm_samples = 0;
  int64_t descriptor_bytes = 0;
  int64_t stats[8] = {0, 0, 0, 0, 0, 0, 0, 0};
  bool sequential_ola = false;
  int last_decoded = -1;
  const char* slot_name[4] = {"-", "-", "-", "-"};
  std::string slot_name_buf[4];
  bool links_ok = false;
  int max_ops = 0, max_ent = 0, max_pass = 0;
  int max_vecs = 0;
  bool block_only = false;
  bool descriptors_only = false;
  bool has_carry_in = false;
  DevBuf dev_copy;
  bool dev_copy_valid = false;
  DevBuf slab3;
  int slab_stride_vecs = 0;
  int slab_cap_vecs = 0;
  bool slabs_ready = false;
  bool slab_host = false;
  const uint4* d_slabs = nullptr;
  int emit_frames = 0;
  bool emit_planar_ok = true;
  int fpw = 1;
  bool ola_all = false;
  int ola_count = 0;
  const int* d_ola_list = nullptr;
  std::vector<nvh::FrameBatch::Gap> gaps;
  DevBuf gap_dev, gap_host;
  std::vector<nvh::FrameBatch::Gap> row_chunks;
  std::vector<nvh::FrameBatch::Segment> segments;
  bool want_seg_flags = false;
  bool seg_table = false;
  DevBuf seg_dev, seg_image;
  int* seg_table_dev() const { return seg_table ? (int*)((uint8_t*)seg_dev.p + 8) : nullptr; }
  int* seg_flags_dev() const { return seg_table ? seg_table_dev() + nframes : nullptr; }
};

struct ReplayLog {
  enum { kPacket = 0, kEnd = 1, kPosition = 2, kSegment = 3, kWindow = 4 };
  struct Event { int kind; int64_t off, len, granule; int flags; };
  std::vector<uint8_t> bytes;
  std::vector<Event> events;
  void clear() { bytes.clear(); events.clear(); }
};

#define NVH_INTERNAL_REPLAY 1000

struct nvh_stream {
  nvh_ctx* ctx = nullptr;
  std::shared_ptr<SharedSetup> shared;
  nvh::Setup& setup;
  DevBuf& arena;
  NvhDevSetup& dev;
  bool& fast_spectrum;
  bool& has_floor0;
  std::unique_ptr<nvh::StreamParser> parser;
  nvh::FrameBatch pending;
  nvh::SlabBatch slab_build;
  DevBuf carry[2];
  int carry_cur = 0;
  DevBuf flags;
  int* seg_table_set = nullptr;
  DevBuf pcm;
  DevBuf h_pcm;
  int clip = 1;
  int has_clipped = 0;
  bool gpu_parse = false;
  DevBuf carry_exec;
  nvh_batch scratch;
  ReplayLog replay;
  std::unique_ptr<nvh::StreamParser> replay_start;
  int replay_error = NVH_OK;
  std::vector<nvh::FrameBatch::Segment> synth_segments;
  std::vector<int32_t> synth_clipped;
  DevBuf h_seg_flags[2];
  std::vector<std::pair<int, int64_t>> replay_errors;
  struct Flight {
    bool on = false;
    hipEvent_t kernels = nullptr, done = nullptr;
    int64_t need = 0;
    int replay_error = NVH_OK;
    std::vector<std::pair<int, int64_t>> replay_errors;
    std::vector<nvh::FrameBatch::Segment> segments;
    int seg_flag_words = 0;
  };
  hipStream_t copy_stream = nullptr;
  DevBuf pcm2[2];
  DevBuf h_flags2;
  Flight flight[2];
  int flight_next = 0, flight_first = 0;
  ~nvh_stream() {
    for (Flight& f : flight) {
      if (f.kernels) (void)hipEventDestroy(f.kernels);
      if (f.done) (void)hipEventDestroy(f.done);
    }
    if (copy_stream) (void)hipStreamDestroy(copy_stream);
  }

  nvh_stream(nvh_ctx* c, std::shared_ptr<SharedSetup> sh)
      : ctx(c), shared(std::move(sh)), setup(shared->setup), arena(shared->arena), dev(shared->dev),
        fast_spectrum(shared->fast_spectrum), has_floor0(shared->has_floor0) {
    BufPool* pool = c ? &c->pool : nullptr;
    carry[0].pool = carry[1].pool = flags.pool = pcm.pool = carry_exec.pool = pcm2[0].pool = pcm2[1].pool = pool;
    h_flags2.host = true;
    h_flags2.pool = c ? &c->hpool : nullptr;
// ... 74 lines not shown
```

nvorbis_amd/csrc/nvh_launch.hip:

```cpp
#include <array>
#include <chrono>

#include "nvh_internal.h"

static int collect_parse_result(nvh_stream* s, nvh_batch* b, const NvhParseResult* d_res);
static bool slab_shape_ok(const nvh_batch* b);
static bool slab_size_ok(const nvh_batch* b);
static void assign_emission(nvh_stream* s, nvh_batch* b, nvh::FrameBatch& P, int fpw, std::vector<int>& ola_list);
static int batch_upload_frames(nvh_stream* s, nvh_batch* b);

void replay_note(nvh_stream* s, int kind, const uint8_t* data, int len, int64_t granule, int flags) {
  if (!s->gpu_parse) return;
  if (s->replay.events.empty()) s->replay_start.reset(new nvh::StreamParser(*s->parser));
  ReplayLog::Event e{kind, (int64_t)s->replay.bytes.size(), (int64_t)len, granule, flags};
  if (kind == ReplayLog::kPacket && len > 0) s->replay.bytes.insert(s->replay.bytes.end(), data, data + len);
  s->replay.events.push_back(e);
}

void replay_note_window(nvh_stream* s, int64_t skip, int64_t take, int64_t pitch) {
  if (!s->gpu_parse) return;
  if (s->replay.events.empty()) s->replay_start.reset(new nvh::StreamParser(*s->parser));
  s->replay.events.push_back(ReplayLog::Event{ReplayLog::kWindow, skip, take, pitch, 0});
}

// ... 201 lines not shown
                         (int)nf, (NvhFrame*)(base + o_fr), (NvhChan*)(base + o_ch), (NvhResPass*)(base + o_ps), (NvhResOp*)(base + o_op),
                         (uint16_t*)(base + o_lk), (uint16_t*)(base + o_en), (uint16_t*)(base + o_po), (int*)(base + o_sc),
                         (NvhParseResult*)(base + o_rs), lanes, (int)sub_words, 0, (uint4*)b->slab3.p,
                         sorted_parse ? (const int*)(base + o_od) : (const int*)nullptr, (uint32_t*)(base + o_ho) NVH_DBG_LAUNCH);
      pkt_words = -1;
    }
    hipLaunchKernelGGL(cur ? k_parse_slab_c : uni ? k_parse_slab_u : slab_mode ? (in_lds ? k_parse_slab : k_parse_slab_g) : (in_lds ? k_parse : k_parse_g),
                       dim3(pblocks), dim3(64 * kParseWaves), parse_lds, st, T,
                       (const uint8_t*)(base + o_pk), (const NvhPacketRef*)(base + o_rf),
                       (int)nf, (NvhFrame*)(base + o_fr), (NvhChan*)(base + o_ch), (NvhResPass*)(base + o_ps), (NvhResOp*)(base + o_op),
                       (uint16_t*)(base + o_lk), (uint16_t*)(base + o_en), (uint16_t*)(base + o_po), (int*)(base + o_sc),
                       (NvhParseResult*)(base + o_rs), lanes, scratch_words, pkt_words, slab_mode ? (uint4*)b->slab3.p : (uint4*)nullptr,
                       sorted_parse ? (const int*)(base + o_od) : (const int*)nullptr, (uint32_t*)(base + o_ho) NVH_DBG_LAUNCH);
    if (cur) {
      constexpr int kTailWaves = 4;
      const size_t tail_lds = ((size_t)T.meta_words + 3 + (size_t)kTailWaves * (NVH_SP_FLOOR_SCRATCH_WORDS + 1) + 8) * sizeof(uint32_t);
      hipLaunchKernelGGL(k_parse_slab_t, dim3((unsigned)((nf + kTailWaves - 1) / kTailWaves)), dim3(64 * kTailWaves), tail_lds, st, T,
                         (const uint8_t*)(base + o_pk), (const NvhPacketRef*)(base + o_rf),
                         (int)nf, (NvhFrame*)(base + o_fr), (NvhChan*)(base + o_ch), (NvhResPass*)(base + o_ps), (NvhResOp*)(base + o_op),
                         (uint16_t*)(base + o_lk), (uint16_t*)(base + o_en), (uint16_t*)(base + o_po), (int*)(base + o_sc),
                         (NvhParseResult*)(base + o_rs), 1, 0, 0, (uint4*)b->slab3.p, (const int*)nullptr, (uint32_t*)(base + o_ho) NVH_DBG_LAUNCH);
    }
    uint32_t* ce = (uint32_t*)s->carry_exec.p;
    hipLaunchKernelGGL(k_parse_links, dim3(blocks), dim3(64), 0, st, (int)nf, ch, (NvhFrame*)(base + o_fr), (NvhChan*)(base + o_ch),
                       (const uint32_t*)(ce + s->carry_cur), ce + (s->carry_cur ^ 1), b->last_decoded, (NvhParseResult*)(base + o_rs),
                       slab_mode ? (uint4*)b->slab3.p : (uint4*)nullptr, (int)T.slab_stride_vecs);
    HIP_TRY(hipGetLastError());
  }
  auto t_c = tnow();
  rc = collect_parse_result(s, b, (const NvhParseResult*)(base + o_rs));
  auto t_d = tnow();
  if (tprint) {
    auto ms = [](std::chrono::steady_clock::time_point a, std::chrono::steady_clock::time_point b) {
      return std::chrono::duration<double, std::milli>(b - a).count();
    };
    fprintf(stderr, "batch_upload_gpu: host prep %.2f ms, enqueue %.2f ms, wait for k_parse %.2f ms\n", ms(t_a, t_b), ms(t_b, t_c), ms(t_c, t_d));
  }
  if (rc != NVH_OK) return rc;
  size_t plane = (size_t)ch * (size_t)s->setup.block1 * sizeof(float);
  rc = b->work.reserve(std::max<size_t>((size_t)b->nframes, 1) * plane);
  if (rc != NVH_OK) return rc;
  if ((rc = poison_planes(s, b, std::max<size_t>((size_t)b->nframes, 1) * plane)) != NVH_OK) return rc;
  if (slab_mode) {
    size_t cap = std::max<size_t>((size_t)b->max_vecs, (size_t)s->setup.block1 / 64 + 8);
    b->slab_cap_vecs = (int)((cap + 3) & ~(size_t)3);
    b->slabs_ready = true;
  } else {
    b->slab_stride_vecs = b->slab_cap_vecs = 0;
  }
  P.clear();
  s->parser->begin_batch();
  return NVH_OK;
}

static int collect_parse_result(nvh_stream* s, nvh_batch* b, const NvhParseResult* d_res) {
  hipStream_t st = s->ctx->stream;
  int rc = s->h_pcm.reserve(sizeof(NvhParseResult));
  if (rc != NVH_OK) return rc;
  NvhParseResult* r = (NvhParseResult*)s->h_pcm.p;
  if (nvh_toggles().copy_upload) {
    HIP_TRY(hipMemcpyAsync(r, d_res, sizeof *r, hipMemcpyDeviceToHost, st));
  } else {
    static_assert(sizeof(NvhParseResult) % 4 == 0 && sizeof(NvhParseResult) <= 256, "k_parse_result_out: one word per lane");
    void* r_dev = nullptr;
    HIP_TRY(hipHostGetDevicePointer(&r_dev, r, 0));
    hipLaunchKernelGGL(k_parse_result_out, dim3(1), dim3(64), 0, st, d_res, (NvhParseResult*)r_dev);
    HIP_TRY(hipGetLastError());
  }
  HIP_TRY(nvh_wait_stream(s->ctx, st));
  b->max_ops = r->max_ops;
  b->max_ent = r->max_ent;
  b->max_pass = r->max_pass;
  b->links_ok = r->links_ok != 0;
  b->max_vecs = r->max_vecs;
  b->ola_all = r->emit_ok == 0;
  if (r->err_frame != 0x7FFFFFFF) return NVH_INTERNAL_REPLAY;
  return NVH_OK;
}

static void assign_emission(nvh_stream* s, nvh_batch* b, nvh::FrameBatch& P, int fpw, std::vector<int>& ola_list) {
  ola_list.clear();
  b->emit_frames = 0;
  b->fpw = 1;
  {
    const int ch = s->setup.channels;
    const bool narrow = ch <= 2 && s->setup.block1 <= 2048 && !s->shared->slab_general;
    const bool wide_emit = !narrow && !s->shared->slab_general && ch <= NVH_SLAB_MAX_CH && s->setup.block1 <= 4096 && !nvh_toggles().no_emit8;
    const bool can = !nvh_toggles().no_emit && (narrow || wide_emit) && !P.sequential_ola && s->setup.block0 >= 256;
    const unsigned all_ch = (1u << ch) - 1u;
    const bool gp = s->gpu_parse;
    auto full = [&](uint32_t m) { return gp || (m & all_ch) == all_ch; };
    const int nf = (int)P.frames.size();
    auto steady = [&](int g) {
      if (!can || g < 1 || g >= nf) return false;
      const NvhFrame& fr = P.frames[(size_t)g];
      const NvhFrame& pv = P.frames[(size_t)g - 1];
      const int half = fr.n >> 1;
      return fr.n >= 256 && pv.n == fr.n && fr.ov_frame == g - 1 && fr.ov_n == fr.n && fr.start == 0 && fr.emit_start == 0 &&
             fr.emit_count == half && fr.ov_src == half && fr.ov_len == half && full(fr.exec_mask) &&
             full(fr.ov_exec_mask) && full(pv.exec_mask) && ((fr.out_pos * ch) & 3) == 0 &&
             fr.out_pos >= 0 && fr.out_pos < 0x7FFFFFFFll && fr.window_off < 0x7FFFFFFFu;
    };
    auto pairable = [&](int g) {
      if (!can || g < 1 || g >= nf) return false;
      const NvhFrame& fr = P.frames[(size_t)g];
      const NvhFrame& pv = P.frames[(size_t)g - 1];
      if (fr.n < 256 || pv.n < 256) return false;
      const int m = fr.n < pv.n ? fr.n : pv.n, half = fr.n >> 1;
      return fr.ov_frame == g - 1 && fr.ov_n == pv.n && fr.ov_window_off == pv.window_off && fr.start == (fr.n >> 2) - (m >> 2) &&
             fr.ov_len == (m >> 1) && fr.ov_src == 3 * (pv.n >> 2) - (m >> 2) && fr.emit_start == fr.start &&
             fr.emit_count == fr.valid - fr.start && fr.valid >= half && fr.valid <= half + (fr.n >> 2) && (fr.valid & 63) == 0 &&
             full(fr.exec_mask) && full(fr.ov_exec_mask) && full(pv.exec_mask) && ((fr.out_pos * ch) & 3) == 0 &&
             fr.out_pos >= 0 && fr.out_pos < 0x7FFFFFFFll && fr.window_off < 0x7FFFFFFFu;
    };
    if (narrow && can && fpw > 1) b->fpw = fpw;
    const int gw = b->fpw;
    auto emits = [&](int g) { return gw > 1 ? pairable(g) : steady(g); };
    for (int g = 0; g < nf; g++) {
      NvhFrame& fr = P.frames[(size_t)g];
      fr.emit_flags = 0;
      const int k = g % gw;
      const bool second_launch = ((g / gw) & 1) == 0;
      if (emits(g)) {
        fr.emit_flags |= NVH_EMIT_DONE;
        if (k > 0 || second_launch) fr.emit_flags |= NVH_EMIT_SELF;
        b->emit_frames++;
      }
      if ((k < gw - 1 || second_launch) && emits(g + 1)) fr.emit_flags |= NVH_EMIT_NEXT;
    }
    if (can && nf > 0) {
      NvhFrame& fr = P.frames[0];
      const int half = fr.n >> 1;
      const bool tail_ok = gw > 1 ? (fr.emit_count == fr.valid - fr.start && fr.valid >= half && fr.valid <= half + (fr.n >> 2) && (fr.valid & 63) == 0)
                                  : fr.emit_count == half;
      if (fr.n >= 256 && fr.ov_frame == -2 && fr.ov_n == fr.n && fr.start == 0 && fr.emit_start == 0 && tail_ok &&
          fr.ov_src == half && fr.ov_len == half && full(fr.exec_mask) && ((fr.out_pos * ch) & 3) == 0 &&
          fr.out_pos >= 0 && fr.out_pos < 0x7FFFFFFFll) {
        fr.emit_flags |= NVH_EMIT_SELF | NVH_EMIT_SELF_CARRY | NVH_EMIT_DONE;
        b->emit_frames++;
      }
    }
    {
      int decoded = 0;
      for (const NvhFrame& fr : P.frames) decoded += fr.n != 0;
      if (!nvh_toggles().emit_always && (long long)b->emit_frames * 8 < (long long)decoded * 7) {
        for (NvhFrame& fr : P.frames) fr.emit_flags = 0;
        b->emit_frames = 0;
        b->fpw = 1;
      }
    }
    int last = -1;
    for (int i = nf - 1; i >= 0; --i)
      if (P.frames[(size_t)i].n != 0) { last = i; break; }
    if (b->emit_frames > 0 && last >= 0 && P.frames[(size_t)last].n >= 256) P.frames[(size_t)last].emit_flags |= NVH_EMIT_CARRY_OUT;
    b->emit_planar_ok = true;
    for (const NvhFrame& fr : P.frames)
      if ((fr.emit_flags & NVH_EMIT_DONE) && (fr.out_pos & 3) != 0) b->emit_planar_ok = false;
    for (int g = 0; g < nf; g++) {
      const NvhFrame& fr = P.frames[(size_t)g];
      if ((fr.emit_count > 0 && !(fr.emit_flags & NVH_EMIT_DONE)) || (g == last && !(fr.emit_flags & NVH_EMIT_CARRY_OUT))) ola_list.push_back(g);
    }
  }
}

static const int64_t kZeroChunkSamples = 4096;
static int64_t zero_chunk_samples() {
  const int kib = nvh_toggles().zero_chunk_kib;
  return kib > 0 ? (int64_t)kib * 256 : kZeroChunkSamples;
}

static int upload_gaps(nvh_stream* s, nvh_batch* b) {
  b->row_chunks.clear();
  const int64_t chunk = zero_chunk_samples();
  size_t keep = 0;
  for (const nvh::FrameBatch::Gap& g : b->gaps) {
    if (g.len <= chunk) { b->gaps[keep++] = g; continue; }
    for (int64_t at = 0; at < g.len; at += chunk) b->row_chunks.push_back({g.pos + at, std::min(chunk, g.len - at)});
  }
  b->gaps.resize(keep);
  if (b->gaps.empty() && b->row_chunks.empty()) return NVH_OK;
  static_assert(sizeof(nvh::FrameBatch::Gap) == 2 * sizeof(long long), "k_zero_gaps reads {position, length} pairs");
  const size_t gap_bytes = b->gaps.size() * sizeof(nvh::FrameBatch::Gap), row_bytes = b->row_chunks.size() * sizeof(nvh::FrameBatch::Gap);
  const size_t bytes = gap_bytes + row_bytes;
  int rc = b->gap_dev.reserve(bytes);
  if (rc == NVH_OK) rc = b->gap_host.reserve(bytes);
  if (rc != NVH_OK) return rc;
  if (gap_bytes) std::memcpy(b->gap_host.p, b->gaps.data(), gap_bytes);
  if (row_bytes) std::memcpy((uint8_t*)b->gap_host.p + gap_bytes, b->row_chunks.data(), row_bytes);
  HIP_TRY(hipMemcpyAsync(b->gap_dev.p, b->gap_host.p, bytes, hipMemcpyHostToDevice, s->ctx->stream));
  return NVH_OK;
}

static int upload_seg_table(nvh_stream* s, nvh_batch* b) {
  if (!b->seg_table) return NVH_OK;
  const size_t bytes = 8 + ((size_t)b->nframes + b->segments.size()) * sizeof(int32_t);
  int rc = b->seg_dev.reserve(bytes);
  if (rc != NVH_OK) return rc;
  int* table = b->seg_table_dev();
  std::memcpy(b->seg_image.p, &table, sizeof table);
  HIP_TRY(hipMemcpyAsync(b->seg_dev.p, b->seg_image.p, bytes, hipMemcpyHostToDevice, s->ctx->stream));
  return NVH_OK;
}

static int build_seg_table(nvh_batch* b, const nvh::FrameBatch& P) {
  b->seg_table = false;
  if (!b->want_seg_flags || b->segments.size() < 2 || P.frames.empty()) return NVH_OK;
  const size_t nf = P.frames.size(), ns = b->segments.size();
  int rc = b->seg_image.reserve(8 + (nf + ns) * sizeof(int32_t));
  if (rc != NVH_OK) return rc;
  int32_t* idx = (int32_t*)((uint8_t*)b->seg_image.p + 8);
  size_t slot = 0;
  for (size_t f = 0; f < nf; f++) {
    const NvhFrame& fr = P.frames[f];
    if (fr.emit_count > 0) {
      while (slot + 1 < ns && (int64_t)fr.out_pos >= b->segments[slot].end) slot++;
      if ((int64_t)fr.out_pos < b->segments[slot].begin || (int64_t)fr.out_pos + fr.emit_count > b->segments[slot].end) return NVH_ERR_RUNTIME;
    }
    idx[f] = (int32_t)(nf + (fr.emit_count > 0 ? slot : 0));
  }
  std::memset(idx + nf, 0, ns * sizeof(int32_t));
  b->seg_table = true;
  return NVH_OK;
}

int batch_upload(nvh_stream* s, nvh_batch* b) {
  int rc = batch_upload_frames(s, b);
  if (rc == NVH_OK) rc = upload_gaps(s, b);
  return rc != NVH_OK ? rc : upload_seg_table(s, b);
}

static int batch_upload_frames(nvh_stream* s, nvh_batch* b) {
  nvh::FrameBatch& P = s->pending;
  b->s = s;
  if (P.frames.empty()) {
    b->nframes = b->chan_frames = 0;
    b->pcm_samples = P.pcm_samples;
    b->segments = P.closed_segments;
    b->segments.push_back({s->parser->segment(), P.segment_begin, P.pcm_samples});
    b->seg_table = false;
    b->gaps = P.gaps;
    b->last_decoded = -1;
    b->ola_count = 0;
    s->replay.clear();
    P.clear();
    s->parser->begin_batch();
    return NVH_OK;
  }
// ... 8 lines not shown
  b->last_decoded = -1;
  b->max_ops = b->max_ent = b->max_pass = 0;
  b->slabs_ready = false;
  b->slab_host = false;
  b->d_slabs = nullptr;
  b->slab_stride_vecs = b->slab_cap_vecs = 0;
  b->links_ok = P.links_ok && P.op_link.size() == P.ops.size();
  for (const NvhFrame& fr : P.frames) {
    if ((int)fr.op_count > b->max_ops) b->max_ops = (int)fr.op_count;
    if ((int)fr.ent_count > b->max_ent) b->max_ent = (int)fr.ent_count;
    if ((int)(fr.pass_end - fr.pass_begin) > b->max_pass) b->max_pass = (int)(fr.pass_end - fr.pass_begin);
    if (fr.chan_off != (uint32_t)((size_t)(&fr - P.frames.data()) * (size_t)s->setup.channels)) return NVH_ERR_RUNTIME;
  }
  for (int i = b->nframes - 1; i >= 0; --i)
    if (P.frames[(size_t)i].n != 0) {
      b->last_decoded = i;
      break;
    }

  std::vector<int> ola_list;
  assign_emission(s, b, P, nvh_toggles().fpw, ola_list);
  b->ola_count = (int)ola_list.size();
  b->d_ola_list = nullptr;
  b->ola_all = false;

  b->stats[0] = (int64_t)P.frames.size(); b->stats[1] = (int64_t)P.chans.size(); b->stats[2] = (int64_t)P.passes.size();
  b->stats[3] = (int64_t)P.ops.size(); b->stats[4] = (int64_t)P.entries.size(); b->stats[5] = (int64_t)P.posts.size();
  b->stats[6] = (int64_t)P.coeffs.size();
  if (s->gpu_parse) {
    if (b->fpw > 1) {
      b->slab_stride_vecs = b->slab_cap_vecs = s->shared->parse.slab_stride_vecs;
      if (!slab_size_ok(b)) assign_emission(s, b, P, 1, ola_list);
      b->ola_count = (int)ola_list.size();
    }
    int rc = batch_upload_gpu(s, b, ola_list);
    if (rc != NVH_INTERNAL_REPLAY) {
      if (rc == NVH_OK) s->replay.clear();
      return rc;
    }
    if ((rc = replay_on_host(s)) != NVH_OK) return rc;
    s->gpu_parse = false;
    rc = batch_upload_frames(s, b);
    s->gpu_parse = true;
    s->replay.clear();
    return rc;
  }
  if (slab_shape_ok(b)) {
    nvh::SlabBatch& SB = s->slab_build;
    int rc = nvh::build_slabs(s->setup, s->shared->slab, P, SB);
    if (rc != NVH_OK && rc != NVH_ERR_UNSUPPORTED) return rc;
    if (rc == NVH_OK) {
      size_t stride = std::max<size_t>(SB.max_vecs, (size_t)s->setup.block1 / 64 + 8);
      stride = (stride + 3) & ~(size_t)3;
      b->slab_stride_vecs = b->slab_cap_vecs = (int)stride;
      b->slab_host = true;
      if (!slab_size_ok(b) && b->fpw > 1) {
        assign_emission(s, b, P, 1, ola_list);
        b->ola_count = (int)ola_list.size();
        rc = nvh::build_slabs(s->setup, s->shared->slab, P, SB);
        if (rc != NVH_OK) return rc;
      }
      if (!slab_size_ok(b)) b->slab_host = false;
    }
    if (b->slab_host) {
      const size_t nf = P.frames.size(), stride = (size_t)b->slab_stride_vecs;
      auto al = [](size_t v) { return (v + 255) & ~(size_t)255; };
      const size_t o_fr = 0;
      const size_t o_ch = al(o_fr + std::max<size_t>(nf, 1) * sizeof(NvhFrame));
      const size_t o_ol = al(o_ch + std::max<size_t>(P.chans.size(), 1) * sizeof(NvhChan));
      const size_t o_sl = al(o_ol + std::max<size_t>(ola_list.size(), 1) * sizeof(int));
      const size_t total = al(o_sl + nf * stride * 16 + 4096);
      if ((rc = b->blob.reserve(total)) != NVH_OK) return rc;
      if ((rc = b->h_blob.reserve(total)) != NVH_OK) return rc;
      uint8_t* h = (uint8_t*)b->h_blob.p;
      if (nf) std::memcpy(h + o_fr, P.frames.data(), nf * sizeof(NvhFrame));
      if (!P.chans.empty()) std::memcpy(h + o_ch, P.chans.data(), P.chans.size() * sizeof(NvhChan));
      if (!ola_list.empty()) std::memcpy(h + o_ol, ola_list.data(), ola_list.size() * sizeof(int));
      int64_t slab_bytes = 0;
      for (size_t f = 0; f < nf; f++) {
        const size_t v = (size_t)(SB.first[f + 1] - SB.first[f]);
        std::memcpy(h + o_sl + f * stride * 16, &SB.data[SB.first[f]], v * 16);
        slab_bytes += (int64_t)v * 16;
      }
      b->descriptor_bytes = (int64_t)(nf * sizeof(NvhFrame) + P.chans.size() * sizeof(NvhChan)) + slab_bytes;
      hipStream_t st = s->ctx->stream;
      HIP_TRY(hipMemcpyAsync(b->blob.p, h, o_sl + nf * stride * 16, hipMemcpyHostToDevice, st));
      const uint8_t* base = (const uint8_t*)b->blob.p;
      b->dev.frames = (const NvhFrame*)(base + o_fr);
      b->dev.chans = (const NvhChan*)(base + o_ch);
      b->dev.passes = nullptr; b->dev.ops = nullptr; b->dev.op_link = nullptr; b->dev.entries = nullptr; b->dev.posts = nullptr; b->dev.coeffs = nullptr;
      b->d_ola_list = (const int*)(base + o_ol);
      b->d_slabs = (const uint4*)(base + o_sl);
      b->dev.nframes = b->nframes;
      b->dev.pad = 0;
      b->dev_copy_valid = false;
      b->slabs_ready = true;
      const size_t plane = (size_t)s->setup.channels * (size_t)s->setup.block1 * sizeof(float);
      if ((rc = b->work.reserve(std::max<size_t>((size_t)b->nframes, 1) * plane)) != NVH_OK) return rc;
      if ((rc = poison_planes(s, b, std::max<size_t>((size_t)b->nframes, 1) * plane)) != NVH_OK) return rc;
      P.clear();
      s->parser->begin_batch();
      return NVH_OK;
    }
  }
  auto pad1 = [](size_t n) { return n ? n : (size_t)1; };
  static const uint8_t dummy[64] = {0};
  struct Piece { const void* src; size_t n, off; };
  std::vector<Piece> pieces;
  size_t total = 0;
  auto add = [&](const void* src, size_t count, size_t elem) {
    const size_t n = pad1(count) * elem;
    total = (total + 15) / 16 * 16;
    pieces.push_back({count ? src : (const void*)dummy, count ? n : (n < sizeof dummy ? n : sizeof dummy), total});
    total += n;
    return pieces.back().off;
  };
  size_t o_fr = add(P.frames.data(), P.frames.size(), sizeof(NvhFrame));
  size_t o_ch = add(P.chans.data(), P.chans.size(), sizeof(NvhChan));
  size_t o_ps = add(P.passes.data(), P.passes.size(), sizeof(NvhResPass));
  size_t o_op = add(P.ops.data(), P.ops.size(), sizeof(NvhResOp));
  size_t o_lk = add(P.op_link.data(), P.op_link.size(), sizeof(uint16_t));
  size_t o_en = add(P.entries.data(), P.entries.size(), sizeof(uint16_t));
  size_t o_po = add(P.posts.data(), P.posts.size(), sizeof(uint16_t));
  size_t o_co = add(P.coeffs.data(), P.coeffs.size(), sizeof(float));
  size_t o_ol = add(ola_list.data(), ola_list.size(), sizeof(int));
  total += 64;
  b->descriptor_bytes = (int64_t)(P.frames.size() * sizeof(NvhFrame) + P.chans.size() * sizeof(NvhChan) +
                                  P.passes.size() * sizeof(NvhResPass) + P.ops.size() * (sizeof(NvhResOp) + sizeof(uint16_t)) +
                                  P.entries.size() * 2 + P.posts.size() * 2 + P.coeffs.size() * 4);
  int rc = b->blob.reserve(total);
  if (rc != NVH_OK) return rc;
  if ((rc = b->h_blob.reserve(total)) != NVH_OK) return rc;
  for (const Piece& pc : pieces) std::memcpy((uint8_t*)b->h_blob.p + pc.off, pc.src, pc.n);
  hipStream_t st = s->ctx->stream;
  HIP_TRY(hipMemcpyAsync(b->blob.p, b->h_blob.p, total, hipMemcpyHostToDevice, st));
  const uint8_t* base = (const uint8_t*)b->blob.p;
  b->dev.frames = (const NvhFrame*)(base + o_fr);
  b->dev.chans = (const NvhChan*)(base + o_ch);
  b->dev.passes = (const NvhResPass*)(base + o_ps);
  b->dev.ops = (const NvhResOp*)(base + o_op);
  b->dev.op_link = (const uint16_t*)(base + o_lk);
  b->dev.entries = (const uint16_t*)(base + o_en);
  b->dev.posts = (const uint16_t*)(base + o_po);
  b->dev.coeffs = (const float*)(base + o_co);
  b->d_ola_list = (const int*)(base + o_ol);
  b->dev.nframes = b->nframes;
  b->dev.pad = 0;
  b->dev_copy_valid = false;

  size_t plane = (size_t)s->setup.channels * (size_t)s->setup.block1 * sizeof(float);
  rc = b->work.reserve(pad1((size_t)b->nframes) * plane);
  if (rc != NVH_OK) return rc;
  if ((rc = poison_planes(s, b, pad1((size_t)b->nframes) * plane)) != NVH_OK) return rc;
  P.clear();
  s->parser->begin_batch();
  return NVH_OK;
}

static int upload_dev_copy(nvh_batch* b, hipStream_t st) {
  if (b->dev_copy_valid && b->dev_copy.p) return NVH_OK;
  int rc = b->dev_copy.reserve(sizeof(NvhDevBatch));
  if (rc != NVH_OK) return rc;
  HIP_TRY(hipMemcpyAsync(b->dev_copy.p, &b->dev, sizeof(NvhDevBatch), hipMemcpyHostToDevice, st));
  b->dev_copy_valid = true;
  return NVH_OK;
}
// ... 119 lines not shown
    const std::string was = b->slot_name[3];
    b->slot_name_buf[3] = was == "-" ? std::string("k_zero_rows") : was + "+k_zero_rows";
    b->slot_name[3] = b->slot_name_buf[3].c_str();
  }
}

int batch_launch(nvh_batch* b, const float* carry, float* carry_out, void* d_pcm, bool timing, float* kernel_ms, hipEvent_t* ext_ev,
                 PcmOut out) {
  nvh_stream* s = b->s;
  hipStream_t st = s->ctx->stream;
  const int ch = s->setup.channels;
  if (b->nframes == 0) {
    if (b->gaps.empty() && b->row_chunks.empty()) return NVH_OK;
    for (int k = 0; k < 4; k++) b->slot_name[k] = "-";
    if (ch == 1 && !out.mapped()) out.plane_stride = 0, out.mix = NVH_MIX_NONE;
    if (d_pcm && !b->block_only) launch_gap_fill(b, out, d_pcm, st);
    HIP_TRY(hipGetLastError());
    return NVH_OK;
  }
  if (ch == 1 && !out.mapped()) out.plane_stride = 0, out.mix = NVH_MIX_NONE;
  const bool planar = out.planar();
  const int64_t plane_stride = out.plane_stride;
  const bool planar_emit = out.mono() || (out.mapped() && !planar)
                               ? (((uintptr_t)d_pcm & 15u) == 0 && b->emit_planar_ok)
                               : !planar || (((uintptr_t)d_pcm & 15u) == 0 && (plane_stride & 3) == 0 &&
                                             plane_stride <= 0x7FFFFFFFll && b->emit_planar_ok);
  const char* sfx = with_pcm_twins(out, [](auto t) { return t.sfx; });
  auto ola_stride = [&](auto t) {
    if constexpr (decltype(t)::layout == NVH_LAYOUT_PLANAR) return (long long)plane_stride;
    else if constexpr (decltype(t)::layout == NVH_LAYOUT_INTERLEAVED_MAP) return out.map;
    else if constexpr (decltype(t)::layout == NVH_LAYOUT_PLANAR_MAP) return NvhStrideMap{(long long)plane_stride, out.map};
    else return NvhNoStride();
  };
  float* work = (float*)b->work.p;
  int* flags = (int*)s->flags.p;
  if (int* table = b->seg_table_dev(); table != s->seg_table_set) {
    if (table) HIP_TRY(hipMemcpyAsync(flags + 2, b->seg_image.p, sizeof table, hipMemcpyHostToDevice, st));
    else HIP_TRY(hipMemsetAsync(flags + 2, 0, sizeof table, st));
    s->seg_table_set = table;
  }
  const size_t lds = (size_t)s->setup.block1 * sizeof(float);
  ScopedEvent sev[5];
  hipEvent_t ev[5] = {nullptr, nullptr, nullptr, nullptr, nullptr};
  if (timing)
    for (int k = 0; k < 5; k++) {
      if (ext_ev) {
        ev[k] = ext_ev[k];
        continue;
      }
      int rc = sev[k].create();
      if (rc != NVH_OK) return rc;
      ev[k] = sev[k].e;
    }
  if (timing) HIP_TRY(hipEventRecord(ev[0], st));
  const NvhToggles& T = nvh_toggles();
  const bool no_compact = T.no_compact, no_fused_imdct = T.no_fused_imdct;
  const bool compact = s->setup.block0 >= 256 && !b->sequential_ola && !no_compact && !b->block_only;
  const bool fast = s->fast_spectrum && b->links_ok;
  bool fuse_imdct = compact && fast && s->setup.block1 <= 2048 && !no_fused_imdct;
  bool fuse_gen8 = false;
  bool slab_done = false;
  bool emitted = false;
  if (b->slabs_ready && compact && !no_fused_imdct) {
    NvhSynthArgs A;
    A.consts = s->shared->synth_consts;
    A.slabs = b->slab_host ? b->d_slabs : (const uint4*)b->slab3.p;
    A.work = work;
    A.err = flags;
    for (int w = 0; w < 2; w++) {
      A.mdct_a[w] = s->dev.mdct_a[w]; A.mdct_b[w] = s->dev.mdct_b[w]; A.mdct_c[w] = s->dev.mdct_c[w]; A.mdct_tw[w] = s->dev.mdct_tw[w];
    }
    A.ipool = s->dev.ipool;
    A.vq = s->dev.vq;
    A.const_vecs = s->shared->synth_const_vecs;
    A.stride_vecs = b->slab_stride_vecs;
    A.cap_vecs = b->slab_cap_vecs;
    A.lds_vecs = (int)slab_lds_vecs(b);
    A.channels = ch;
    A.block1 = s->setup.block1;
    A.f0 = 0; A.fstep = 1;
    A.nframes = b->nframes;
    A.prefetch_prev = 0;
    A.xcd_map = 0;
    A.walk_two = nvh_toggles().no_walk_two ? 0 : 1;
    const bool wide = slab_wide(s);
    emitted = b->emit_frames > 0 && d_pcm != nullptr && !b->block_only && !T.no_emit && !s->shared->slab_general && planar_emit &&
              (wide || !out.mapped());
    A.pcm = emitted ? (float*)d_pcm : nullptr;
    A.windows = s->dev.windows;
    A.clip = s->clip;
    A.plane_stride = planar && planar_emit ? (int)plane_stride : 0;
    A.clipped_flag = flags + 1;
    A.carry = carry;
    A.carry_out = emitted ? carry_out : nullptr;
    A.frames = b->dev.frames;
    const size_t synth_lds = slab_lds_bytes(b) + (size_t)T.lds_pad;
    if (synth_lds > 64 * 1024 && !s->ctx->synth_lds_attr_set) {
      HIP_TRY(hipFuncSetAttribute((const void*)k_synth8, hipFuncAttributeMaxDynamicSharedMemorySize, 160 * 1024));
      HIP_TRY(hipFuncSetAttribute((const void*)k_synth8_g, hipFuncAttributeMaxDynamicSharedMemorySize, 160 * 1024));
      hipError_t attr_err = hipSuccess;
      auto big_lds = [&](auto t) {
        if (attr_err == hipSuccess) attr_err = hipFuncSetAttribute((const void*)t.synth8_emit, hipFuncAttributeMaxDynamicSharedMemorySize, 160 * 1024);
      };
      for_pcm_twins(big_lds);
      for_pcm_map_twins(big_lds);
      HIP_TRY(attr_err);
      s->ctx->synth_lds_attr_set = true;
    }
    if (timing) HIP_TRY(hipEventRecord(ev[1], st));
    b->slot_name[0] = "-";
    const bool narrow_general = !wide && s->shared->slab_general;
    const bool wide_general = wide && s->shared->slab_general;
    b->slot_name[1] = wide ? (wide_general ? "k_synth8_g" : "k_synth8") : (narrow_general ? "k_synth_g" : "k_synth");
    if (wide && emitted) {
      A.fstep = 2;
      A.f0 = 1;
      if (b->nframes > 1) hipLaunchKernelGGL(k_synth8, dim3((unsigned)(b->nframes / 2)), dim3(512), synth_lds, st, A NVH_DBG_LAUNCH);
      A.f0 = 0;
      with_pcm_twins(out, [&](auto t) {
        const dim3 grid((unsigned)((b->nframes + 1) / 2));
        if constexpr (nvh_layout_mapped(decltype(t)::layout)) hipLaunchKernelGGL(t.synth8_emit, grid, dim3(512), synth_lds, st, A, out.map NVH_DBG_LAUNCH);
        else hipLaunchKernelGGL(t.synth8_emit, grid, dim3(512), synth_lds, st, A NVH_DBG_LAUNCH);
      });
    } else if (wide_general) hipLaunchKernelGGL(k_synth8_g, dim3((unsigned)b->nframes), dim3(512), synth_lds, st, A NVH_DBG_LAUNCH);
    else if (wide) hipLaunchKernelGGL(k_synth8, dim3((unsigned)b->nframes), dim3(512), synth_lds, st, A NVH_DBG_LAUNCH);
    else if (narrow_general) hipLaunchKernelGGL(k_synth_g, dim3((unsigned)b->nframes), dim3(256), synth_lds, st, A NVH_DBG_LAUNCH);
    else if (!emitted) hipLaunchKernelGGL(k_synth, dim3((unsigned)b->nframes), dim3(NVH_SYNTH_NT), synth_lds, st, A NVH_DBG_LAUNCH);
    else if (b->fpw > 1) {
      const int gw = b->fpw, ngroups = (b->nframes + gw - 1) / gw;
      if (synth_lds > 64 * 1024 && !s->ctx->group_lds_attr_set) {
        hipError_t attr_err = hipSuccess;
        for_pcm_twins([&](auto t) {
          for (const void* k : {(const void*)t.group2, (const void*)t.group4})
            if (attr_err == hipSuccess) attr_err = hipFuncSetAttribute(k, hipFuncAttributeMaxDynamicSharedMemorySize, 160 * 1024);
        });
        HIP_TRY(attr_err);
        s->ctx->group_lds_attr_set = true;
      }
      auto kern = with_unmapped_twins(out, [gw](auto t) { return gw == 2 ? t.group2 : t.group4; });
      const unsigned nt = gw == 2 ? 256u : 512u;
      if (T.debug_occ) {
        int nb = -1;
        hipError_t oe = hipOccupancyMaxActiveBlocksPerMultiprocessor(&nb, (const void*)kern, (int)nt, synth_lds);
        hipFuncAttributes fa;
        (void)hipFuncGetAttributes(&fa, (const void*)kern);
        fprintf(stderr, "frame groups of %d: %u threads, lds %zu B (constants %d, slab area %d, largest slab %d vecs), occupancy %d WG/CU (err %d), regs %d\n",
                gw, nt, synth_lds, A.const_vecs, A.lds_vecs, A.cap_vecs, nb, (int)oe, fa.numRegs);
      }
      A.fstep = 2 * gw;
      A.f0 = gw;
      static const bool group_prefetch = std::getenv("NVH_GROUP_PREFETCH") != nullptr;
      A.prefetch_prev = group_prefetch ? 1 : 0;
      if (ngroups / 2 > 0) hipLaunchKernelGGL(kern, dim3((unsigned)(ngroups / 2)), dim3(nt), synth_lds, st, A NVH_DBG_LAUNCH);
      A.f0 = 0;
      A.prefetch_prev = 0;
      hipLaunchKernelGGL(kern, dim3((unsigned)((ngroups + 1) / 2)), dim3(nt), synth_lds, st, A NVH_DBG_LAUNCH);
    } else {
      A.fstep = 2;
      A.f0 = 1;
      A.prefetch_prev = nvh_toggles().no_prefetch ? 0 : 1;
      A.xcd_map = nvh_toggles().xcd_map ? 1 : 0;
      if (b->nframes > 1) {
        if (b->last_decoded >= 0 && (b->last_decoded & 1))
          hipLaunchKernelGGL(k_synth_tail, dim3((unsigned)(b->nframes / 2)), dim3(NVH_SYNTH_NT), synth_lds, st, A NVH_DBG_LAUNCH);
        else
          hipLaunchKernelGGL(k_synth, dim3((unsigned)(b->nframes / 2)), dim3(NVH_SYNTH_NT), synth_lds, st, A NVH_DBG_LAUNCH);
      }
// ... 177 lines not shown
```

nvorbis_amd/native.py:

```python
import ctypes as C
import os

from . import build as _build

OK = 0
ERR_INVALID_DATA, ERR_ARGUMENT, ERR_RUNTIME, ERR_NOMEM = -1, -2, -3, -4
ERR_NOT_VORBIS, ERR_DEVICE, ERR_UNSUPPORTED, ERR_NO_GPU = -5, -6, -7, -8
PKT_EOS, PKT_RESYNC = 1, 2
PCM_F32, PCM_S16 = 0, 1
MIX_NONE, MIX_MONO = 0, 1

_ERRNAMES = {
    ERR_INVALID_DATA: "InvalidDataException", ERR_ARGUMENT: "ArgumentOutOfRangeException",
    ERR_RUNTIME: "runtime fault (IndexOutOfRange/NullReference class)", ERR_NOMEM: "out of memory",
    ERR_NOT_VORBIS: "not a Vorbis stream", ERR_DEVICE: "HIP error", ERR_UNSUPPORTED: "unsupported stream",
    ERR_NO_GPU: "no HIP device (there is no CPU fallback)",
}


class NvhError(RuntimeError):
    def __init__(self, code, where=""):
        self.code = code
        extra = ""
        if code == ERR_DEVICE:
# ... 79 lines not shown
SIGNATURES = {
    "nvh_version": (C.c_char_p, []),
    "nvh_last_hip_error": (C.c_int, []),
    "nvh_device_count": (C.c_int, []),
    "nvh_ctx_create": (C.c_int, [C.c_int, _vpp]),
    "nvh_ctx_destroy": (None, [_vp]),
    "nvh_ctx_set_hip_stream": (C.c_int, [_vp, _vp]),
    "nvh_ctx_synchronize": (C.c_int, [_vp]),
    "nvh_ctx_set_parse_lanes": (C.c_int, [_vp, C.c_int]),
    "nvh_dev_alloc": (C.c_int, [_vp, C.c_size_t, _vpp]),
    "nvh_dev_free": (None, [_vp, _vp]),
    "nvh_dev_upload": (C.c_int, [_vp, _vp, _vp, C.c_size_t]),
    "nvh_dev_download": (C.c_int, [_vp, _vp, _vp, C.c_size_t]),
    "nvh_measure_copy": (C.c_int, [_vp, _vp, _vp, C.c_size_t, C.c_int, _f32p]),
    "nvh_stream_bitrates": (C.c_int, [_vp, _ip, _ip, _ip]),
    "nvh_mdct_reverse": (C.c_int, [_vp, C.c_int, C.c_int, _vp, C.c_int64]),
    "nvh_inverse_couple": (C.c_int, [_vp, _vp, _vp, C.c_int]),
    "nvh_mode_decode": (C.c_int, [_vp, _vp, C.c_int, _vp] + [C.POINTER(C.c_int)] * 5),
    "nvh_residue_decode": (C.c_int, [_vp, C.c_int, _vp, C.c_int, C.c_int, C.c_int, C.c_int, _vp, C.POINTER(C.c_int)]),
    "nvh_window_apply": (C.c_int, [_vp, C.c_int, C.c_int, C.c_int, C.c_int, _vp, C.c_int64]),
    "nvh_overlap_buffers": (C.c_int, [_vp, _vp, _vp, C.c_int, C.c_int, C.c_int, C.c_int, C.c_int64]),
    "nvh_copy_buffer": (C.c_int, [_vp, _vp, C.c_int, C.c_int, C.c_int, C.c_int64, _vp, C.c_int, C.POINTER(C.c_int)]),
    "nvh_stream_mode_info": (C.c_int, [_vp, C.c_int] + [C.POINTER(C.c_int)] * 3),
    "nvh_stream_codebook_info": (C.c_int, [_vp, C.c_int] + [C.POINTER(C.c_int)] * 7),
    "nvh_stream_codebook_tables": (C.c_int, [_vp, C.c_int, _vp, _vp, _vp, _vp]),
    "nvh_stream_parse_book_info": (C.c_int, [_vp, C.c_int] + [C.POINTER(C.c_int)] * 6),
    "nvh_stream_position_state": (C.c_int, [_vp, C.POINTER(C.c_int), C.POINTER(C.c_int64)]),
    "nvh_stream_set_position_state": (C.c_int, [_vp, C.c_int, C.c_int64]),
    "nvh_stream_drop_pending": (C.c_int, [_vp]),
    "nvh_stream_packet_sample_count": (C.c_int, [_vp, _vp, C.c_int, C.c_int, C.POINTER(C.c_int)]),
    "nvh_stream_reset": (C.c_int, [_vp]),
    "nvh_stream_index_packets": (C.c_int, [_vp, _vp, _vp, _vp, _vp, C.c_int, _vp, _vp, _vp, C.POINTER(C.c_int64)]),
    "nvh_floor0_apply": (C.c_int, [_vp, C.c_int, C.c_int, C.c_int, _vp, _vp, C.c_int, _vp, C.c_int64, _vp]),
    "nvh_floor1_apply": (C.c_int, [_vp, C.c_int, C.c_int, C.c_int, _vp, _vp, _vp, C.c_int64, _vp]),
    "nvh_stream_floor_info": (C.c_int, [_vp, C.c_int] + [C.POINTER(C.c_int)] * 3),
    "nvh_mdct_tables": (C.c_int, [C.c_int, _vp, _vp, _vp, _vp]),
    "nvh_calc_window": (C.c_int, [C.c_int, C.c_int, C.c_int, _vp]),
    "nvh_calc_overlap": (C.c_int, [C.c_int, C.c_int, C.c_int, _ip, _ip, _ip]),
    "nvh_stream_open": (C.c_int, [_vp, _vp, C.c_int, _vp, C.c_int, _vp, C.c_int, _vpp]),
    "nvh_stream_close": (None, [_vp]),
    "nvh_stream_info": (C.c_int, [_vp, _ip, _ip, _ip, _ip]),
    "nvh_stream_set_clip": (C.c_int, [_vp, C.c_int]),
    "nvh_pinned_alloc": (C.c_int, [C.c_size_t, C.POINTER(C.c_void_p)]),
    "nvh_pinned_free": (None, [_vp]),
    "nvh_stream_set_gpu_parse": (C.c_int, [_vp, C.c_int]),
    "nvh_stream_has_clipped": (C.c_int, [_vp, _ip]),
    "nvh_stream_position": (C.c_int, [_vp, _i64p, _i64p, _ip]),
    "nvh_stream_push_packet": (C.c_int, [_vp, _vp, C.c_int, C.c_int64, C.c_int]),
    "nvh_stream_push_packets": (C.c_int, [_vp, _vp, _vp, _vp, _vp, C.c_int, C.c_int, C.POINTER(C.c_int)]),
    "nvh_stream_push_end": (C.c_int, [_vp]),
    "nvh_stream_pending": (C.c_int, [_vp, _ip, _i64p]),
    "nvh_stream_next_segment": (C.c_int, [_vp, C.c_int]),
    "nvh_stream_segment_window": (C.c_int, [_vp, C.c_int64, C.c_int64, C.c_int64]),
    "nvh_stream_pending_segments": (C.c_int, [_vp, _i64p, _i64p, _i64p, C.c_int, _ip]),
    "nvh_stream_synth_segments": (C.c_int, [_vp, _i64p, _i64p, _i64p, C.c_int, _ip]),
    "nvh_stream_synth_segments_clipped": (C.c_int, [_vp, _ip, C.c_int, _ip]),
    "nvh_stream_pending_geometry": (C.c_int, [_vp, _vp, C.c_int]),
    "nvh_stream_pending_slabs": (C.c_int, [_vp, _vp, C.c_int64, _i64p, _vp, C.c_int]),
    "nvh_stream_lattice_pool": (C.c_int, [_vp, _vp, C.c_int64, _i64p]),
    "nvh_stream_vq_pool": (C.c_int, [_vp, _vp, C.c_int64, _i64p]),
    "nvh_stream_synth_out": (C.c_int, [_vp, C.POINTER(PcmOut), _vp, _vp, _i64p]),
    "nvh_stream_synth_begin_out": (C.c_int, [_vp, C.POINTER(PcmOut), _vp, _i64p]),
    "nvh_batch_synth_out": (C.c_int, [_vp, C.POINTER(PcmOut), _vp]),
    "nvh_stream_synth_begin": (C.c_int, [_vp, _vp, C.c_int64, _i64p]),
    "nvh_stream_synth_end": (C.c_int, [_vp, _i64p]),
    "nvh_stream_synth": (C.c_int, [_vp, _vp, _vp, C.c_int64, _i64p]),
    "nvh_stream_synth_pcm": (C.c_int, [_vp, C.c_int, _vp, _vp, C.c_int64, _i64p]),
    "nvh_stream_synth_begin_pcm": (C.c_int, [_vp, C.c_int, _vp, C.c_int64, _i64p]),
    "nvh_stream_synth_planar": (C.c_int, [_vp, C.c_int, _vp, _vp, C.c_int64, _i64p]),
    "nvh_stream_synth_begin_planar": (C.c_int, [_vp, C.c_int, _vp, C.c_int64, _i64p]),
    "nvh_stream_synth_mix": (C.c_int, [_vp, C.c_int, C.c_int, _vp, _vp, C.c_int64, _i64p]),
    "nvh_stream_synth_begin_mix": (C.c_int, [_vp, C.c_int, C.c_int, _vp, C.c_int64, _i64p]),
    "nvh_channel_map_wave": (C.c_int, [C.c_int, _i32p]),
    "nvh_stream_synth_map": (C.c_int, [_vp, C.c_int, _i32p, C.c_int, _vp, _vp, C.c_int64, _i64p]),
    "nvh_stream_synth_begin_map": (C.c_int, [_vp, C.c_int, _i32p, C.c_int, _vp, C.c_int64, _i64p]),
    "nvh_stream_synth_planar_map": (C.c_int, [_vp, C.c_int, _i32p, C.c_int, _vp, _vp, C.c_int64, _i64p]),
    "nvh_stream_synth_begin_planar_map": (C.c_int, [_vp, C.c_int, _i32p, C.c_int, _vp, C.c_int64, _i64p]),
    "nvh_stream_parse_errors": (C.c_int, [_vp, _i32p, _i64p, C.c_int, _ip]),
    "nvh_batch_upload": (C.c_int, [_vp, _vpp]),
    "nvh_batch_info": (C.c_int, [_vp, _ip, _ip, _i64p, _i64p]),
    "nvh_batch_stats": (C.c_int, [_vp, _i64p]),
    "nvh_batch_kernels": (C.c_int, [_vp, C.c_char_p, C.c_int]),
    "nvh_stream_kernels": (C.c_int, [_vp, C.c_char_p, C.c_int]),
    "nvh_batch_synth": (C.c_int, [_vp, _vp, C.c_int64]),
    "nvh_batch_synth_pcm": (C.c_int, [_vp, C.c_int, _vp, C.c_int64]),
    "nvh_batch_synth_planar": (C.c_int, [_vp, C.c_int, _vp, C.c_int64]),
    "nvh_batch_synth_mix": (C.c_int, [_vp, C.c_int, C.c_int, _vp, C.c_int64]),
    "nvh_batch_synth_map": (C.c_int, [_vp, C.c_int, _i32p, C.c_int, _vp, C.c_int64]),
    "nvh_batch_synth_planar_map": (C.c_int, [_vp, C.c_int, _i32p, C.c_int, _vp, C.c_int64]),
    "nvh_batch_time": (C.c_int, [_vp, _vp, C.c_int64, C.c_int, _f32p, _f32p]),
    "nvh_batch_free": (None, [_vp]),
    "nvh_ogg_demux": (C.c_int, [_vp, C.c_size_t, _vp, C.c_int64, _vp, _vp, _vp, C.c_int, _ip, _i64p]),
    "nvh_ogg_demux_forward": (C.c_int, [_vp, C.c_size_t, C.c_int, _vp, C.c_int64, _vp, _vp, _vp, C.c_int, _ip, _i64p, _ip]),
    "nvh_ogg_index_open": (C.c_int, [_vp, C.c_size_t, C.c_int, C.POINTER(_vp)]),
    "nvh_ogg_index_close": (None, [_vp]),
    "nvh_ogg_index_info": (C.c_int, [_vp, _ip, _ip, _ip, _i64p, _ip]),
    "nvh_ogg_index_page": (C.c_int, [_vp, C.c_int, _i64p, _ip, _ip, _ip]),
    "nvh_ogg_seek": (C.c_int, [_vp, _vp, C.c_int64, C.c_int, _i64p, _i64p]),
    "nvh_ogg_demux_stream": (C.c_int, [_vp, C.c_size_t, C.c_int, _vp, C.c_int64, _vp, _vp, _vp, C.c_int, _ip, _i64p, _ip]),
    "nvh_ogg_index_packets": (C.c_int, [_vp, C.c_size_t, C.c_int, _vp, C.c_int64, _vp, _vp, _vp, C.c_int, _ip, _i64p, _i64p, _ip]),
    "nvh_resample_plan": (C.c_int, [C.c_int, C.c_int, _ip, _ip, _ip, _i64p]),
    "nvh_resample_taps": (C.c_int, [C.c_int, C.c_int, _vp, C.c_int64, _i64p]),
    "nvh_resample_rows": (C.c_int, [_vp, C.POINTER(ResampleDesc), _vp, _vp, _vp, _vp, _vp, _vp, _vp]),
    "nvh_resample_route": (C.c_int, [C.POINTER(ResampleDesc), _i64p]),
    "nvh_mel_plan": (C.c_int, [C.POINTER(MelDesc), _i64p, _i64p, _i64p]),
    "nvh_mel_tables": (C.c_int, [C.POINTER(MelDesc), _vp, _vp, _vp, C.c_int64, C.c_int64, C.c_int64, _i64p, _i64p, _i64p]),
    "nvh_mel_rows": (C.c_int, [_vp, C.POINTER(MelDesc), _vp, _vp, _vp]),
    "nvh_mel_front_check": (C.c_int, [C.POINTER(MelDesc), C.POINTER(MelFront)]),
    "nvh_mel_tables_front": (C.c_int, [C.POINTER(MelDesc), C.POINTER(MelFront), _vp, _vp, _vp, C.c_int64, C.c_int64, C.c_int64, _i64p, _i64p,
                                       _i64p]),
    "nvh_mel_rows_front": (C.c_int, [_vp, C.POINTER(MelDesc), C.POINTER(MelFront), _vp, _vp, _vp]),
    "nvh_mel_route": (C.c_int, [C.POINTER(MelDesc), C.POINTER(MelFront), _i64p]),
    "nvh_fnorm_check": (C.c_int, [C.POINTER(FnormDesc)]),
    "nvh_fnorm_rows": (C.c_int, [_vp, C.POINTER(FnormDesc), _vp, _vp, _vp]),
    "nvh_fnorm_route": (C.c_int, [C.POINTER(FnormDesc), _i64p]),
    "nvh_cep_check": (C.c_int, [C.POINTER(CepDesc)]),
    "nvh_cep_plan": (C.c_int, [C.POINTER(CepDesc), _i64p, _i64p]),
    "nvh_cep_tables": (C.c_int, [C.POINTER(CepDesc), _vp, _vp, C.c_int64, C.c_int64, _i64p, _i64p]),
    "nvh_cep_rows": (C.c_int, [_vp, C.POINTER(CepDesc), _vp, _vp, _vp]),
    "nvh_cep_route": (C.c_int, [C.POINTER(CepDesc), _i64p]),
    "nvh_comm_unique_id": (C.c_int, [_vp]),
    "nvh_comm_create": (C.c_int, [_vp, _vp, C.c_int, C.c_int, C.POINTER(_vp)]),
    "nvh_comm_destroy": (None, [_vp]),
    "nvh_comm_info": (C.c_int, [_vp, _ip, _ip]),
    "nvh_comm_allgather_i64": (C.c_int, [_vp, _i64p, C.c_int, _i64p]),
    "nvh_comm_gather_pcm": (C.c_int, [_vp, _vp, C.c_int64, _vp, _i64p, C.c_int, C.c_int]),
}

_lib = None


def lib_path():
    return os.environ.get("NVH_LIB") or os.path.join(os.path.dirname(os.path.abspath(__file__)), "libnvorbis_hip.so")


def lib():
    global _lib
    if _lib is None:
        try:
            import torch
        except ImportError:
            pass
        path = lib_path()
        if os.environ.get("NVH_LIB"):
            if not os.environ.get("NVH_ALLOW_STALE") and _build.embedded_hash(path) != _build.source_hash():
                raise RuntimeError("%s was built from other sources (has %s, tree is %s): rebuild it or set NVH_ALLOW_STALE=1"
                                   % (path, _build.embedded_hash(path), _build.source_hash()))
        elif _build.needs_build(path):
            import sys
            sys.stderr.write("nvorbis_amd: %s is missing or stale (has %s, sources are %s): building\n"
                             % (path, _build.embedded_hash(path), _build.source_hash()))
            _build.build(force=True)
            if _build.needs_build(path):
                raise RuntimeError("libnvorbis_hip.so does not carry the hash of its sources after a rebuild")
        handle = C.CDLL(path)
        for name, (res, args) in SIGNATURES.items():
            fn = getattr(handle, name)
            fn.restype = res
            fn.argtypes = args
        ver = handle.nvh_version().decode()
        if not os.environ.get("NVH_ALLOW_STALE") and ("nvh-src-hash=" + _build.source_hash()) not in ver:
            raise RuntimeError("loaded %s reports '%s', sources are %s" % (path, ver, _build.source_hash()))
        _lib = handle
    return _lib


# ... 9 lines not shown
```

nvorbis_amd/reader.py:

```python
import ctypes as C
import threading

import numpy as np

from . import native
from .native import check, lib


_PCM_FORMATS = {np.dtype(np.float32): native.PCM_F32, np.dtype(np.int16): native.PCM_S16}
_SAMPLE_FORMATS = {"f32": np.float32, "s16": np.int16}


def _pcm_format(dtype):
    dt = np.dtype(dtype)
    if dt not in _PCM_FORMATS:
        raise ValueError("PCM dtype must be float32 or int16, not %s" % dt)
    return _PCM_FORMATS[dt], dt


_LAYOUTS = ("interleaved", "planar")


def _layout(name):
    if not isinstance(name, str) or name not in _LAYOUTS:
# ... 238 lines not shown

    def synchronize(self):
        check(lib().nvh_ctx_synchronize(self._h), "nvh_ctx_synchronize")

    def set_parse_lanes(self, lanes):
        check(lib().nvh_ctx_set_parse_lanes(self._h, int(lanes)), "nvh_ctx_set_parse_lanes")

    def mdct_reverse(self, n, batch, d_ptr, stride):
        check(lib().nvh_mdct_reverse(self._h, int(n), int(batch), C.c_void_p(d_ptr), int(stride)), "nvh_mdct_reverse")

    def overlap_buffers(self, d_previous, d_next, prev_start, prev_stop, next_start, channels, plane_stride):
        check(lib().nvh_overlap_buffers(self._h, C.c_void_p(d_previous), C.c_void_p(d_next), int(prev_start), int(prev_stop),
                                        int(next_start), int(channels), int(plane_stride)), "nvh_overlap_buffers")

    def copy_buffer(self, d_planes, start, count, channels, plane_stride, d_target, clip=True):
        clipped = C.c_int(0)
        check(lib().nvh_copy_buffer(self._h, C.c_void_p(d_planes), int(start), int(count), int(channels), int(plane_stride),
                                    C.c_void_p(d_target), 1 if clip else 0, C.byref(clipped)), "nvh_copy_buffer")
        return bool(clipped.value)

    def inverse_couple(self, d_magnitude, d_angle, count):
        check(lib().nvh_inverse_couple(self._h, C.c_void_p(d_magnitude), C.c_void_p(d_angle), int(count)), "nvh_inverse_couple")

    def resample_rows(self, desc, d_src, d_dst, origin, start, valid, dst_row=None, d_clipped=None):
        o, s, v = (_row_array("resample_rows", "the per-row arrays hold", a, desc.rows) for a in (origin, start, valid))
        r = _row_array("resample_rows", "the per-row arrays hold", dst_row, desc.rows, np.int32)
        check(lib().nvh_resample_rows(self._h, C.byref(desc), C.c_void_p(d_src), C.c_void_p(d_dst), o.ctypes.data, s.ctypes.data,
                                      v.ctypes.data, None if r is None else r.ctypes.data,
                                      None if d_clipped is None else C.c_void_p(d_clipped)), "nvh_resample_rows")

    def mel_rows(self, desc, d_src, d_dst, valid=None, front=None):
        v = _row_array("mel_rows", "valid holds", valid, desc.rows)
        if front is None:
            check(lib().nvh_mel_rows(self._h, C.byref(desc), C.c_void_p(d_src), C.c_void_p(d_dst), None if v is None else v.ctypes.data),
                  "nvh_mel_rows")
        else:
            check(lib().nvh_mel_rows_front(self._h, C.byref(desc), C.byref(front), C.c_void_p(d_src), C.c_void_p(d_dst),
                                           None if v is None else v.ctypes.data), "nvh_mel_rows_front")

    def fnorm_rows(self, desc, d_src, d_dst, valid_frames=None):
        v = _row_array("fnorm_rows", "valid_frames holds", valid_frames, desc.rows)
        check(lib().nvh_fnorm_rows(self._h, C.byref(desc), C.c_void_p(d_src), C.c_void_p(d_dst), None if v is None else v.ctypes.data),
              "nvh_fnorm_rows")

    def cep_rows(self, desc, d_src, d_dst, valid_frames=None):
        v = _row_array("cep_rows", "valid_frames holds", valid_frames, desc.rows)
        check(lib().nvh_cep_rows(self._h, C.byref(desc), C.c_void_p(d_src), C.c_void_p(d_dst), None if v is None else v.ctypes.data),
              "nvh_cep_rows")

    def close(self):
        if self._h:
            lib().nvh_ctx_destroy(self._h)
            self._h = C.c_void_p()

    def __del__(self):
        try:
            self.close()
        except Exception:
            pass


class Batch:

    def __init__(self, handle, stream):
        self._h = handle
        self._stream = stream
        self.channels = stream.channels
        fr, cf = C.c_int(0), C.c_int(0)
        smp, db = C.c_int64(0), C.c_int64(0)
        check(lib().nvh_batch_info(self._h, C.byref(fr), C.byref(cf), C.byref(smp), C.byref(db)), "nvh_batch_info")
        self.frames, self.chan_frames, self.samples, self.descriptor_bytes = fr.value, cf.value, smp.value, db.value

    def stats(self):
        out = (C.c_int64 * 8)()
        check(lib().nvh_batch_stats(self._h, out), "nvh_batch_stats")
        keys = ["frames", "chan_frames", "passes", "ops", "entries", "posts", "coeffs", "reserved"]
        return {k: out[i] for i, k in enumerate(keys)}

    def kernels(self):
        buf = C.create_string_buffer(256)
        check(lib().nvh_batch_kernels(self._h, buf, 256), "nvh_batch_kernels")
        return buf.value.decode().split(",")

    def synth(self, d_pcm_ptr, capacity, dtype=np.float32, plane_stride=None, mix=None, channel_map=None):
        d, _, _, _ = _pcm_out(dtype, plane_stride is not None, mix, channel_map, self._stream.channels)
        d.extent = int(capacity if plane_stride is None else plane_stride)
        check(lib().nvh_batch_synth_out(self._h, C.byref(d), C.c_void_p(d_pcm_ptr)), "nvh_batch_synth_out")

    def time(self, d_pcm_ptr, capacity, iters, per_kernel=True):
        total = C.c_float(0)
        km = (C.c_float * 4)()
        check(lib().nvh_batch_time(self._h, C.c_void_p(d_pcm_ptr), int(capacity), int(iters), C.byref(total),
                                   km if per_kernel else None), "nvh_batch_time")
        return total.value, [km[i] for i in range(4)]

    def free(self):
        if self._h:
            lib().nvh_batch_free(self._h)
            self._h = None

    def __del__(self):
        try:
            self.free()
        except Exception:
            pass


class _PinnedBuffer:

    def __init__(self):
        self._ptr, self._cap, self._bytes = None, 0, None

    def get(self, n, dt):
        nbytes = n * dt.itemsize
        if self._cap < nbytes:
            cap = max(nbytes, 2 * self._cap)
            self.free()
            p = C.c_void_p()
            check(lib().nvh_pinned_alloc(cap, C.byref(p)), "nvh_pinned_alloc")
            self._ptr, self._cap = p, cap
            self._bytes = np.ctypeslib.as_array(C.cast(p, C.POINTER(C.c_uint8)), shape=(cap,))
        return self._bytes[:self._cap - self._cap % dt.itemsize].view(dt)

    def free(self):
        if self._ptr:
            self._bytes = None
            lib().nvh_pinned_free(self._ptr)
            self._ptr, self._cap = None, 0


class Stream:

    def __init__(self, ctx, id_pkt, comment_pkt, setup_pkt):
        self._ctx = ctx
        self._pinned = _PinnedBuffer()
        self._flight_bufs = (_PinnedBuffer(), _PinnedBuffer())
        self._flight_out = [None, None]
        self._flight_per_channel = [False, False]
        self._flight_channels = [0, 0]
        self._pipe_next = self._pipe_first = self._pipe_out = 0
        self._h = C.c_void_p()
        check(lib().nvh_stream_open(ctx._h if ctx is not None else None, id_pkt, len(id_pkt), comment_pkt,
                                    len(comment_pkt) if comment_pkt is not None else 0, setup_pkt, len(setup_pkt),
                                    C.byref(self._h)), "nvh_stream_open")
        ch, sr, b0, b1 = C.c_int(0), C.c_int(0), C.c_int(0), C.c_int(0)
        check(lib().nvh_stream_info(self._h, C.byref(ch), C.byref(sr), C.byref(b0), C.byref(b1)), "nvh_stream_info")
        self.channels, self.sample_rate, self.block0, self.block1 = ch.value, sr.value, b0.value, b1.value
        self.parse_errors = []

    def bitrates(self):
        u, n, l = C.c_int(0), C.c_int(0), C.c_int(0)
        check(lib().nvh_stream_bitrates(self._h, C.byref(u), C.byref(n), C.byref(l)), "nvh_stream_bitrates")
        return u.value, n.value, l.value

    def push_packet(self, data, granule=-1, flags=0):
        check(lib().nvh_stream_push_packet(self._h, data, len(data), int(granule), int(flags)), "nvh_stream_push_packet")

    def push_packets(self, pa, first, max_packets):
        took = C.c_int(0)
        n = len(pa) - first
        rc = lib().nvh_stream_push_packets(self._h, pa.data.ctypes.data, pa.offsets[first:].ctypes.data,
                                           pa.granules[first:].ctypes.data, pa.flags[first:].ctypes.data, int(n),
                                           int(max_packets), C.byref(took))
        if rc != native.OK:
            e = native.NvhError(rc, "nvh_stream_push_packets")
            e.consumed = took.value + 1
            raise e
        return took.value

    def push_end(self):
        check(lib().nvh_stream_push_end(self._h), "nvh_stream_push_end")

    def pending(self):
        fr, smp = C.c_int(0), C.c_int64(0)
        check(lib().nvh_stream_pending(self._h, C.byref(fr), C.byref(smp)), "nvh_stream_pending")
        return fr.value, smp.value

    def next_segment(self, align=1):
        check(lib().nvh_stream_next_segment(self._h, int(align)), "nvh_stream_next_segment")

    def segment_window(self, skip=0, take=-1, pitch=0):
        check(lib().nvh_stream_segment_window(self._h, int(skip), int(take), int(pitch)), "nvh_stream_segment_window")

    def pending_segments(self):
        return self._segments(lib().nvh_stream_pending_segments, "nvh_stream_pending_segments")

    def synth_segments(self):
        return self._segments(lib().nvh_stream_synth_segments, "nvh_stream_synth_segments")

    def synth_segments_clipped(self):
        n = C.c_int(0)
        lib().nvh_stream_synth_segments_clipped(self._h, None, 0, C.byref(n))
        out = np.zeros(max(n.value, 1), dtype=np.int32)
        check(lib().nvh_stream_synth_segments_clipped(self._h, out.ctypes.data_as(C.POINTER(C.c_int)), out.shape[0], C.byref(n)),
              "nvh_stream_synth_segments_clipped")
        return out[:n.value] != 0

    def _segments(self, fn, where):
        n = C.c_int(0)
        fn(self._h, None, None, None, 0, C.byref(n))
        out = np.zeros((3, max(n.value, 1)), dtype=np.int64)
        i64 = C.POINTER(C.c_int64)
        check(fn(self._h, out[0].ctypes.data_as(i64), out[1].ctypes.data_as(i64), out[2].ctypes.data_as(i64), out.shape[1], C.byref(n)), where)
        return np.ascontiguousarray(out[:, :n.value].T)

    def pending_geometry(self):
        fr, _ = self.pending()
        out = np.zeros((max(fr, 1), 8), dtype=np.int32)
        check(lib().nvh_stream_pending_geometry(self._h, out.ctypes.data, max(fr, 1)), "nvh_stream_pending_geometry")
        return out[:fr]

    def kernels(self):
        buf = C.create_string_buffer(256)
        check(lib().nvh_stream_kernels(self._h, buf, 256), "nvh_stream_kernels")
        return buf.value.decode().split(",")

    def pending_slabs(self):
        fr, _ = self.pending()
        need = C.c_int64(0)
        first = np.zeros(fr + 1, dtype=np.uint32)
        rc = lib().nvh_stream_pending_slabs(self._h, None, 0, C.byref(need), first.ctypes.data, fr + 1)
        if rc not in (0, -2):
            check(rc, "nvh_stream_pending_slabs")
        buf = np.zeros(max(need.value // 4, 4), dtype=np.uint32)
        check(lib().nvh_stream_pending_slabs(self._h, buf.ctypes.data, buf.nbytes, C.byref(need), first.ctypes.data, fr + 1),
              "nvh_stream_pending_slabs")
        return buf[:need.value // 4], first

    def lattice_pool(self):
        need = C.c_int64(0)
        lib().nvh_stream_lattice_pool(self._h, None, 0, C.byref(need))
        buf = np.zeros(max(int(need.value), 1), np.uint32)
        check(lib().nvh_stream_lattice_pool(self._h, buf.ctypes.data, buf.size, C.byref(need)), "nvh_stream_lattice_pool")
        return buf[:int(need.value)]

    def vq_pool(self):
        need = C.c_int64(0)
        lib().nvh_stream_vq_pool(self._h, None, 0, C.byref(need))
        buf = np.zeros(max(int(need.value), 1), np.float32)
        check(lib().nvh_stream_vq_pool(self._h, buf.ctypes.data, buf.size, C.byref(need)), "nvh_stream_vq_pool")
        return buf[:int(need.value)]

    def position(self):
        pos, em, eos = C.c_int64(0), C.c_int64(0), C.c_int(0)
        check(lib().nvh_stream_position(self._h, C.byref(pos), C.byref(em), C.byref(eos)), "nvh_stream_position")
        return pos.value, em.value, bool(eos.value)

    def position_state(self):
        h, p = C.c_int(0), C.c_int64(0)
        check(lib().nvh_stream_position_state(self._h, C.byref(h), C.byref(p)), "nvh_stream_position_state")
        return bool(h.value), p.value

    def set_position_state(self, has_position, position):
        check(lib().nvh_stream_set_position_state(self._h, 1 if has_position else 0, int(position)), "nvh_stream_set_position_state")

    def index_packets(self, pa, first=3):
        n = max(0, len(pa) - first)
        pos, em, st = np.zeros(max(n, 1), np.int64), np.zeros(max(n, 1), np.int64), np.zeros(max(n, 1), np.uint8)
        total = C.c_int64(0)
        check(lib().nvh_stream_index_packets(self._h, pa.data.ctypes.data, pa.offsets[first:].ctypes.data if n else pa.offsets.ctypes.data,
                                             pa.granules[first:].ctypes.data if n else None, pa.flags[first:].ctypes.data if n else None,
                                             n, pos.ctypes.data, em.ctypes.data, st.ctypes.data, C.byref(total)), "nvh_stream_index_packets")
        return pos[:n], em[:n], st[:n], total.value

    def index_total(self, pa, first=3):
        n = max(0, len(pa) - first)
        total = C.c_int64(0)
        check(lib().nvh_stream_index_packets(self._h, pa.data.ctypes.data, pa.offsets[first:].ctypes.data if n else pa.offsets.ctypes.data,
                                             pa.granules[first:].ctypes.data if n else None, pa.flags[first:].ctypes.data if n else None,
                                             n, None, None, None, C.byref(total)), "nvh_stream_index_packets")
        return total.value

    def packet_sample_count(self, packet, is_resync=False):
        n = C.c_int(0)
        check(lib().nvh_stream_packet_sample_count(self._h, packet, len(packet), 1 if is_resync else 0, C.byref(n)),
              "nvh_stream_packet_sample_count")
        return n.value

    def reset(self):
        check(lib().nvh_stream_reset(self._h), "nvh_stream_reset")
        self._pipe_next = self._pipe_first = self._pipe_out = 0

    def drop_pending(self):
        check(lib().nvh_stream_drop_pending(self._h), "nvh_stream_drop_pending")

    def mode_decode(self, packet, d_block):
        dec, bs, a, b, c = C.c_int(0), C.c_int(0), C.c_int(0), C.c_int(0), C.c_int(0)
        check(lib().nvh_mode_decode(self._h, packet, len(packet), C.c_void_p(d_block), C.byref(dec), C.byref(bs), C.byref(a),
                                    C.byref(b), C.byref(c)), "nvh_mode_decode")
        return (bs.value, a.value, b.value, c.value) if dec.value else None

    def residue_decode(self, residue_index, packet, bit_offset, block_size, d_buffer, any_channel_decodes=True):
        bits = C.c_int(0)
        check(lib().nvh_residue_decode(self._h, int(residue_index), packet, len(packet), int(bit_offset),
                                       1 if any_channel_decodes else 0, int(block_size), C.c_void_p(d_buffer), C.byref(bits)),
              "nvh_residue_decode")
        return bits.value

# ... 596 lines not shown
```

Before: 190.8 million frames/s.

## Add specialized steady-state path for stereo long-block frame pairs in synth kernel

Adds a device-side check that detects frame pairs with uniform geometry (stereo, fixed block size, floor1 fused, residue2 geometry, matching emit flags) from the slab headers. Such pairs take a specialized synth_group_steady path with compile-time block size, a lean residue walk using a wave ballot loop, fixed floor mode, and a direct emit loop that skips the generic per-task table. This aims to cut the branching, header re-reads and generic indexing in the common case. It also adds host and API helpers to count steady groups, and enlarges register use by loading all 16 header words per frame.

Result: faster. 209.1 million frames/s, median of 6 (+9.6%).

```diff
diff --git a/include/nvorbis_hip.h b/include/nvorbis_hip.h
--- a/include/nvorbis_hip.h
+++ b/include/nvorbis_hip.h
@@ -152,6 +152,10 @@
 int nvh_batch_stats(const nvh_batch *b, int64_t *out8);
 int nvh_batch_kernels(const nvh_batch *b, char *buf, int cap);
 int nvh_stream_kernels(const nvh_stream *s, char *buf, int cap);
+int nvh_batch_steady_groups(const nvh_batch *b, int *groups);
+int nvh_stream_steady_groups(const nvh_stream *s, int *groups);
+int nvh_stream_pending_steady(const nvh_stream *s, int *groups);
+int nvh_steady_count(const uint32_t *headers, int frames, int channels, int block1, int *groups);
 int nvh_batch_synth_out(nvh_batch *b, const nvh_pcm_out *out, void *d_pcm);
 int nvh_batch_synth(nvh_batch *b, float *d_pcm, int64_t capacity);
 int nvh_batch_synth_pcm(nvh_batch *b, int format, void *d_pcm, int64_t capacity);
diff --git a/nvorbis_amd/csrc/kernels_synth.hip b/nvorbis_amd/csrc/kernels_synth.hip
--- a/nvorbis_amd/csrc/kernels_synth.hip
+++ b/nvorbis_amd/csrc/kernels_synth.hip
@@ -266,7 +266,7 @@
   FloorRef F;
 };
 
-template <int NT>
+template <int NT, bool LEAN = false>
 __device__ __forceinline__ void residue_walk_two(const WalkFrame (&W)[2], const uint32_t* __restrict__ s_lat, int tid) {
   constexpr int G = 8;
   const uint32_t* heads[2];
@@ -303,6 +303,47 @@
 #ifdef NVH_ABL_NO_CHAIN2
     more[0] = more[1] = false;
 #endif
+    if constexpr (LEAN) {
+      float v[2][G];
+#pragma unroll
+      for (int f = 0; f < 2; ++f) {
+        const char* vb = reinterpret_cast<const char*>(s_lat) + ((rec[f].y & 0xFFFu) << 2);
+        const uint2 w = *reinterpret_cast<const uint2*>(ent[f] + ((rec[f].x & 0xFFFFu) << 1) + i0[f]);
+#pragma unroll
+        for (int k = 0; k < 4; ++k) {
+          v[f][k] = *reinterpret_cast<const float*>(vb + ((w.x >> (8 * k)) & 0xFFu));
+          v[f][4 + k] = *reinterpret_cast<const float*>(vb + ((w.y >> (8 * k)) & 0xFFu));
+        }
+      }
+#pragma unroll
+      for (int f = 0; f < 2; ++f) {
+#pragma unroll
+        for (int k = 0; k < G; ++k) a[f][k] = a[f][k] + v[f][k];
+        more[f] = more[f] && (rec[f].y & 0x80000000u) != 0u;
+      }
+      while (__builtin_amdgcn_ballot_w64(more[0] | more[1]) != 0ull) {
+#pragma unroll
+        for (int f = 0; f < 2; ++f)
+          if (more[f]) rec[f] = recs[f][++o[f]];
+#pragma unroll
+        for (int f = 0; f < 2; ++f) {
+          const char* vb = reinterpret_cast<const char*>(s_lat) + ((rec[f].y & 0xFFFu) << 2);
+          const uint2 w = *reinterpret_cast<const uint2*>(ent[f] + ((rec[f].x & 0xFFFFu) << 1) + i0[f]);
+#pragma unroll
+          for (int k = 0; k < 4; ++k) {
+            v[f][k] = *reinterpret_cast<const float*>(vb + ((w.x >> (8 * k)) & 0xFFu));
+            v[f][4 + k] = *reinterpret_cast<const float*>(vb + ((w.y >> (8 * k)) & 0xFFu));
+          }
+        }
+#pragma unroll
+        for (int f = 0; f < 2; ++f) {
+          const uint32_t keep = more[f] ? 0xFFFFFFFFu : 0u;
+#pragma unroll
+          for (int k = 0; k < G; ++k) a[f][k] = a[f][k] + __uint_as_float(__float_as_uint(v[f][k]) & keep);
+          more[f] = more[f] && (rec[f].y & 0x80000000u) != 0u;
+        }
+      }
+    } else
     while (more[0] | more[1]) {
       float v[2][G];
 #pragma unroll
@@ -345,7 +386,7 @@
 #ifdef NVH_ABL_NO_FLOOR2
           if (false) {
 #else
-          if (W[f].F.md[c] == 1) {
+          if (LEAN || W[f].F.md[c] == 1) {
 #endif
             float m[4];
             floor_walk_fx<4>(W[f].F.seg[c], W[f].F.tab[c], W[f].F.s_db, (int)xb, m);
@@ -1473,6 +1514,171 @@
 #undef SY_T
 }
 
+template <typename PCM, int LAYOUT>
+__device__ __forceinline__ void group_emit_task(const NvhSynthArgs& A, const float* smem, unsigned woff, unsigned wpoff, unsigned pos,
+                                                unsigned aoff, unsigned astr, unsigned boff, unsigned bstr, int n, int g, int nch,
+                                                int cbit, int* clipped) {
+  constexpr bool PLANAR = LAYOUT == NVH_LAYOUT_PLANAR, MONO = LAYOUT == NVH_LAYOUT_MONO;
+  const int half = n >> 1, i0 = 4 * g;
+  const float* __restrict__ w = A.windows + woff;
+  const float* __restrict__ wp = A.windows + wpoff;
+  const float4 wf = *reinterpret_cast<const float4*>(w + i0);
+  const float4 wm = *reinterpret_cast<const float4*>(w + (half - 4 - i0));
+  const float4 pf = *reinterpret_cast<const float4*>(wp + i0);
+  const float4 pm = *reinterpret_cast<const float4*>(wp + (half - 4 - i0));
+  float fwd[8], mir[8];
+#pragma unroll
+  for (int c = 0; c < 2; ++c) {
+    if (c < nch) {
+      const float4 a = *reinterpret_cast<const float4*>(smem + aoff + c * astr + i0);
+      const float4 b = *reinterpret_cast<const float4*>(smem + boff + c * bstr + i0);
+      float4 v = make_float4(a.x * wf.x, a.y * wf.y, a.z * wf.z, a.w * wf.w);
+      const float4 tt = make_float4(b.x * pf.x, b.y * pf.y, b.z * pf.z, b.w * pf.w);
+      v.x = v.x + tt.x; v.y = v.y + tt.y; v.z = v.z + tt.z; v.w = v.w + tt.w;
+      float4 u = make_float4(-a.w * wm.x, -a.z * wm.y, -a.y * wm.z, -a.x * wm.w);
+      const float4 r = make_float4(b.w * pm.x, b.z * pm.y, b.y * pm.z, b.x * pm.w);
+      u.x = u.x + r.x; u.y = u.y + r.y; u.z = u.z + r.z; u.w = u.w + r.w;
+      if (!MONO && A.clip) {
+        v.x = clip_value(v.x, clipped, cbit); v.y = clip_value(v.y, clipped, cbit);
+        v.z = clip_value(v.z, clipped, cbit); v.w = clip_value(v.w, clipped, cbit);
+        u.x = clip_value(u.x, clipped, cbit); u.y = clip_value(u.y, clipped, cbit);
+        u.z = clip_value(u.z, clipped, cbit); u.w = clip_value(u.w, clipped, cbit);
+      }
+      if constexpr (PLANAR) {
+        pcm_store_plane(reinterpret_cast<PCM*>(A.pcm) + (long long)pos + (long long)c * A.plane_stride, g, (n >> 3) - 1 - g, v, u);
+      } else {
+        fwd[c] = v.x; fwd[2 + c] = v.y; fwd[4 + c] = v.z; fwd[6 + c] = v.w;
+        mir[c] = u.x; mir[2 + c] = u.y; mir[4 + c] = u.z; mir[6 + c] = u.w;
+      }
+    }
+  }
+  PCM* out = reinterpret_cast<PCM*>(A.pcm) + (long long)pos * (PLANAR || MONO ? 1 : nch);
+  if constexpr (PLANAR) {
+  } else if constexpr (MONO) {
+    pcm_store_plane(out, g, (n >> 3) - 1 - g, mono_mix2(fwd, nch, A.clip, clipped, cbit), mono_mix2(mir, nch, A.clip, clipped, cbit));
+  } else if (nch == 2) {
+    pcm4_t<PCM>* of = reinterpret_cast<pcm4_t<PCM>*>(out) + 2 * (long long)g;
+    pcm4_t<PCM>* om = reinterpret_cast<pcm4_t<PCM>*>(out) + 2 * (long long)((n >> 3) - 1 - g);
+    if constexpr (std::is_same<PCM, int16_t>::value) {
+      pcm_store4x2(of, fwd);
+      pcm_store4x2(om, mir);
+    } else {
+      pcm_store4(of, fwd[0], fwd[1], fwd[2], fwd[3]);
+      pcm_store4(of + 1, fwd[4], fwd[5], fwd[6], fwd[7]);
+      pcm_store4(om, mir[0], mir[1], mir[2], mir[3]);
+      pcm_store4(om + 1, mir[4], mir[5], mir[6], mir[7]);
+    }
+  } else {
+    pcm_store4(reinterpret_cast<pcm4_t<PCM>*>(out) + g, fwd[0], fwd[2], fwd[4], fwd[6]);
+    pcm_store4(reinterpret_cast<pcm4_t<PCM>*>(out) + ((n >> 3) - 1 - g), mir[0], mir[2], mir[4], mir[6]);
+  }
+}
+
+#ifdef NVH_DEBUG
+#define GR_T(k) do { if (dbg && tid == 0 && fa < A.nframes) dbg[(long long)fa * 24 + (k)] = clock64(); } while (0)
+#else
+#define GR_T(k) do { } while (0)
+#endif
+
+template <int LD, typename PCM, int LAYOUT>
+__device__ __forceinline__ void synth_group_steady(const NvhSynthArgs& A, float* smem, const unsigned (&H)[2][NVH_SLAB_HDR_WORDS], bool import,
+                                                   int fa, int tid, int wv, int lane NVH_DBG_PARAMS) {
+  constexpr int NT = 256, n = 1 << LD, half = n >> 1, quarter = n >> 2;
+  constexpr int slice_words = half + (n >> 4), S0 = n, SK = 2 * slice_words;
+  float* s_db = smem;
+  const uint32_t* s_lat = reinterpret_cast<const uint32_t*>(smem + 256);
+  float* slab0 = smem + A.const_vecs * 4;
+  const int slab_words = A.lds_vecs * 4;
+  float* spec0 = slab0 + 2 * slab_words;
+  {
+    WalkFrame W[2];
+#pragma unroll
+    for (int k = 0; k < 2; ++k) {
+      W[k].slab = slab0 + k * slab_words;
+      W[k].nheads = H[k][1] & 0xFFFFu; W[k].off_heads = H[k][2] & 0xFFFFu; W[k].off_rec = H[k][2] >> 16; W[k].off_ent = H[k][3] & 0xFFFFu;
+      W[k].lpc = H[k][4] & 0xFFFFu; W[k].lpc_magic = H[k][5]; W[k].flags = H[k][0] >> 24;
+      W[k].spec = spec0 + k * n; W[k].half = half;
+#pragma unroll
+      for (int c = 0; c < 2; ++c) {
+        const unsigned cw = H[k][8 + c], ns = (cw >> 8) & 0xFFu, oseg = cw >> 16;
+        W[k].F.seg[c] = reinterpret_cast<const uint4*>(W[k].slab + oseg * 4);
+        W[k].F.tab[c] = reinterpret_cast<const uint8_t*>(W[k].slab + (oseg + ns) * 4);
+        W[k].F.md[c] = 1;
+      }
+      W[k].F.s_db = s_db;
+    }
+    residue_walk_two<NT, true>(W, s_lat, tid);
+    GR_T(2); GR_T(3);
+  }
+  __syncthreads();
+  GR_T(4);
+
+  if (import) {
+    constexpr int units = n >> 3;
+    const float* pB = A.work + (long long)(fa - 1) * 2 * n + half;
+    const float* pA = A.work + (long long)(fa + 2) * 2 * n;
+    for (int u0 = wv * 64; u0 < units; u0 += NT) {
+      const int u = u0 + lane, c = u >> (LD - 4), r = u & ((n >> 4) - 1);
+      dma16<kStageAux>(reinterpret_cast<const uint4*>(pB + c * n + 4 * r), smem + 4 * u0);
+      dma16<kStageAux>(reinterpret_cast<const uint4*>(pA + c * n + 4 * r), smem + half + 4 * u0);
+    }
+  }
+
+  {
+    const int k = wv >> 1, c = wv & 1;
+    const unsigned f0w = H[0][0], f1w = H[1][0];
+    const unsigned flags = (k ? f1w : f0w) >> 24;
+    const int sl = (flags & NVH_SLAB_MDCT_SLOT) ? 1 : 0;
+    const float* X = spec0 + k * n + c * half;
+    float* slice = smem + S0 + (k * 2 + c) * slice_words;
+    float4 ca[2] = {make_float4(0.f, 0.f, 0.f, 0.f), make_float4(0.f, 0.f, 0.f, 0.f)}, cb[2] = {ca[0], ca[0]};
+    auto sink = [&](int slot, int, float4 v) {
+      if (slot == 0) ca[0] = v; else if (slot == 2) cb[0] = v; else if (slot == 4) ca[1] = v; else if (slot == 6) cb[1] = v;
+    };
+    imdct_wave_sink<LD, false, decltype(sink), true, true, false, kSynthPFEmit, true>(X, nullptr, slice, A.mdct_a[sl], A.mdct_b[sl], A.mdct_c[sl],
+                                                                                       A.mdct_tw[sl], lane, sink, nullptr, kAblSkip);
+    if (lane < (n >> 5)) {
+      const int i8a = lane, i8b = (n >> 4) - 1 - lane;
+      if (!import) {
+        float* plane = A.work + ((long long)(fa + k) * 2 + c) * n;
+        if (k == 0) {
+          *reinterpret_cast<float4*>(plane + 4 * i8a) = ca[0];
+          *reinterpret_cast<float4*>(plane + 4 * i8b) = ca[1];
+        } else {
+          *reinterpret_cast<float4*>(plane + half + 4 * i8a) = cb[0];
+          *reinterpret_cast<float4*>(plane + half + 4 * i8b) = cb[1];
+        }
+      }
+      *reinterpret_cast<float4*>(slice + 4 * i8a) = ca[0];
+      *reinterpret_cast<float4*>(slice + 4 * i8b) = ca[1];
+      *reinterpret_cast<float4*>(slice + quarter + 4 * i8a) = cb[0];
+      *reinterpret_cast<float4*>(slice + quarter + 4 * i8b) = cb[1];
+    }
+  }
+  GR_T(5);
+  __syncthreads();
+  GR_T(6);
+
+  {
+    constexpr int WPO = 1 << (LD - 10);
+    int clipped = 0;
+    const int r0 = import ? 0 : WPO, r1 = import ? 3 * WPO : 2 * WPO;
+    const unsigned win0 = H[0][10], ovw0 = H[0][11], nxw0 = H[0][12], pos0 = H[0][14], nxp0 = H[0][15];
+    const unsigned win1 = H[1][10], nxw1 = H[1][12], nxp1 = H[1][15];
+    for (int r = r0 + wv; r < r1; r += NT / 64) {
+      const int j = r >> (LD - 10), g = ((r & (WPO - 1)) << 6) + lane;
+      const unsigned woff = j == 0 ? win0 : (j == 1 ? nxw0 : nxw1);
+      const unsigned wpoff = (j == 0 ? ovw0 : (j == 1 ? win0 : win1)) + (unsigned)half;
+      const unsigned pos = j == 0 ? pos0 : (j == 1 ? nxp0 : nxp1);
+      const unsigned aoff = j == 2 ? (unsigned)half : (unsigned)(S0 + j * SK), astr = j == 2 ? (unsigned)quarter : (unsigned)slice_words;
+      const unsigned boff = j == 0 ? 0u : (unsigned)(S0 + (j - 1) * SK + quarter), bstr = j == 0 ? (unsigned)quarter : (unsigned)slice_words;
+      group_emit_task<PCM, LAYOUT>(A, smem, woff, wpoff, pos, aoff, astr, boff, bstr, n, g, 2, 1 << j, &clipped);
+    }
+    if (A.clip) report_clipped<3>(clipped, A.clipped_flag, fa);
+  }
+  GR_T(7);
+}
+
 template <int NT, int FPW, typename PCM = float, int LAYOUT = NVH_LAYOUT_INTERLEAVED>
 __device__ __forceinline__ void synth_group_body(const NvhSynthArgs& A, float* smem NVH_DBG_PARAMS) {
   static_assert(NT / 64 >= 2 * FPW, "one wavefront per (frame, channel) in the transform");
@@ -1480,11 +1686,6 @@
   const int tid = threadIdx.x, wv = __builtin_amdgcn_readfirstlane(tid >> 6), lane = tid & 63;
   const int nch = A.channels;
   const int fa = A.f0 + (int)blockIdx.x * A.fstep;
-#ifdef NVH_DEBUG
-#define GR_T(k) do { if (dbg && tid == 0 && fa < A.nframes) dbg[(long long)fa * 24 + (k)] = clock64(); } while (0)
-#else
-#define GR_T(k) do { } while (0)
-#endif
   GR_T(0);
   const int half_max = A.block1 >> 1, pad_max = A.block1 >> 4;
   float* s_db = smem;
@@ -1498,14 +1699,26 @@
   const int walk_end = A.const_vecs * 4 + FPW * (slab_words + region), xform_end = nch * half_max + FPW * nch * slice_words;
   uint32_t* otab = reinterpret_cast<uint32_t*>(smem + (walk_end > xform_end ? walk_end : xform_end));
   typedef const __attribute__((address_space(4))) uint32_t* const_words;
+  constexpr bool STEADY = FPW == 2 && NT == 256;
   unsigned w0[FPW], w3[FPW];
+  unsigned H[STEADY ? 2 : 1][NVH_SLAB_HDR_WORDS];
 #pragma unroll
   for (int k = 0; k < FPW; ++k) {
     w0[k] = 0u; w3[k] = 0u;
+    if constexpr (STEADY) {
+#pragma unroll
+      for (int i = 0; i < NVH_SLAB_HDR_WORDS; ++i) H[k][i] = 0u;
+    }
     if (fa + k < A.nframes) {
       const uint4* gslab = A.slabs + (long long)(fa + k) * A.stride_vecs;
       const_words gh = (const_words)(unsigned long long)gslab;
-      w0[k] = gh[0]; w3[k] = gh[3];
+      if constexpr (STEADY) {
+#pragma unroll
+        for (int i = 0; i < NVH_SLAB_HDR_WORDS; ++i) H[k][i] = gh[i];
+        w0[k] = H[k][0]; w3[k] = H[k][3];
+      } else {
+        w0[k] = gh[0]; w3[k] = gh[3];
+      }
       if (tid < A.cap_vecs) dma16<kSlabAux>(gslab + tid, slab0 + k * slab_words + wv * 256);
     }
   }
@@ -1545,6 +1758,15 @@
   __syncthreads();
   if (!any) return;
   GR_T(1);
+
+  if constexpr (STEADY) {
+    bool import = false;
+    if ((A.walk_two & 2) && A.pcm != nullptr && nvh_steady_pair(H[0], H[1], nch, A.block1, &import)) {
+      if (A.block1 == 2048) synth_group_steady<11, PCM, LAYOUT>(A, smem, H, import, fa, tid, wv, lane NVH_DBG_ARGS);
+      else synth_group_steady<10, PCM, LAYOUT>(A, smem, H, import, fa, tid, wv, lane NVH_DBG_ARGS);
+      return;
+    }
+  }
 
   auto hdr = [&](int k, int i) { return __builtin_amdgcn_readfirstlane(reinterpret_cast<const uint32_t*>(slab0 + k * slab_words)[i]); };
   {
@@ -1762,60 +1984,7 @@
 #pragma unroll
     for (int jj = 1; jj <= FPW; ++jj) g = j == jj ? t - cnt[jj] : g;
     const uint4 r0 = reinterpret_cast<const uint4*>(otab)[2 * j], r1 = reinterpret_cast<const uint4*>(otab)[2 * j + 1];
-    const int n = (int)r0.w, half = n >> 1, i0 = 4 * g;
-    const int cbit = 1 << j;
-    const float* __restrict__ w = A.windows + r0.x;
-    const float* __restrict__ wp = A.windows + r0.y;
-    const float4 wf = *reinterpret_cast<const float4*>(w + i0);
-    const float4 wm = *reinterpret_cast<const float4*>(w + (half - 4 - i0));
-    const float4 pf = *reinterpret_cast<const float4*>(wp + i0);
-    const float4 pm = *reinterpret_cast<const float4*>(wp + (half - 4 - i0));
-    float fwd[8], mir[8];
-#pragma unroll
-    for (int c = 0; c < 2; ++c) {
-      if (c < nch) {
-        const float4 a = *reinterpret_cast<const float4*>(smem + r1.x + c * r1.y + i0);
-        const float4 b = *reinterpret_cast<const float4*>(smem + r1.z + c * r1.w + i0);
-        float4 v = make_float4(a.x * wf.x, a.y * wf.y, a.z * wf.z, a.w * wf.w);
-        const float4 tt = make_float4(b.x * pf.x, b.y * pf.y, b.z * pf.z, b.w * pf.w);
-        v.x = v.x + tt.x; v.y = v.y + tt.y; v.z = v.z + tt.z; v.w = v.w + tt.w;
-        float4 u = make_float4(-a.w * wm.x, -a.z * wm.y, -a.y * wm.z, -a.x * wm.w);
-        const float4 r = make_float4(b.w * pm.x, b.z * pm.y, b.y * pm.z, b.x * pm.w);
-        u.x = u.x + r.x; u.y = u.y + r.y; u.z = u.z + r.z; u.w = u.w + r.w;
-        if (!MONO && A.clip) {
-          v.x = clip_value(v.x, &clipped, cbit); v.y = clip_value(v.y, &clipped, cbit);
-          v.z = clip_value(v.z, &clipped, cbit); v.w = clip_value(v.w, &clipped, cbit);
-          u.x = clip_value(u.x, &clipped, cbit); u.y = clip_value(u.y, &clipped, cbit);
-          u.z = clip_value(u.z, &clipped, cbit); u.w = clip_value(u.w, &clipped, cbit);
-        }
-        if constexpr (PLANAR) {
-          pcm_store_plane(reinterpret_cast<PCM*>(A.pcm) + (long long)r0.z + (long long)c * A.plane_stride, g, (n >> 3) - 1 - g, v, u);
-        } else {
-          fwd[c] = v.x; fwd[2 + c] = v.y; fwd[4 + c] = v.z; fwd[6 + c] = v.w;
-            mir[c] = u.x; mir[2 + c] = u.y; mir[4 + c] = u.z; mir[6 + c] = u.w;
-        }
-      }
-    }
-    PCM* out = reinterpret_cast<PCM*>(A.pcm) + (long long)r0.z * (PLANAR || MONO ? 1 : nch);
-    if constexpr (PLANAR) {
-    } else if constexpr (MONO) {
-      pcm_store_plane(out, g, (n >> 3) - 1 - g, mono_mix2(fwd, nch, A.clip, &clipped, cbit), mono_mix2(mir, nch, A.clip, &clipped, cbit));
-    } else if (nch == 2) {
-      pcm4_t<PCM>* of = reinterpret_cast<pcm4_t<PCM>*>(out) + 2 * (long long)g;
-      pcm4_t<PCM>* om = reinterpret_cast<pcm4_t<PCM>*>(out) + 2 * (long long)((n >> 3) - 1 - g);
-      if constexpr (std::is_same<PCM, int16_t>::value) {
-        pcm_store4x2(of, fwd);
-        pcm_store4x2(om, mir);
-      } else {
-        pcm_store4(of, fwd[0], fwd[1], fwd[2], fwd[3]);
-        pcm_store4(of + 1, fwd[4], fwd[5], fwd[6], fwd[7]);
-        pcm_store4(om, mir[0], mir[1], mir[2], mir[3]);
-        pcm_store4(om + 1, mir[4], mir[5], mir[6], mir[7]);
-      }
-    } else {
-      pcm_store4(reinterpret_cast<pcm4_t<PCM>*>(out) + g, fwd[0], fwd[2], fwd[4], fwd[6]);
-      pcm_store4(reinterpret_cast<pcm4_t<PCM>*>(out) + ((n >> 3) - 1 - g), mir[0], mir[2], mir[4], mir[6]);
-    }
+    group_emit_task<PCM, LAYOUT>(A, smem, r0.x, r0.y, r0.z, r1.x, r1.y, r1.z, r1.w, (int)r0.w, g, nch, 1 << j, &clipped);
   }
   int fcnt[FPW + 1];
   fcnt[0] = 0;
diff --git a/nvorbis_amd/csrc/nvh_api.hip b/nvorbis_amd/csrc/nvh_api.hip
--- a/nvorbis_amd/csrc/nvh_api.hip
+++ b/nvorbis_amd/csrc/nvh_api.hip
@@ -23,6 +23,7 @@
     x.no_emit8 = on("NVH_NO_EMIT8");
     x.no_prefetch = on("NVH_NO_PREFETCH");
     x.no_walk_two = on("NVH_NO_WALK_TWO");
+    x.no_steady = on("NVH_NO_STEADY");
     x.fpw = std::getenv("NVH_FPW") ? num("NVH_FPW") : 2;
     if (x.fpw != 1 && x.fpw != 2 && x.fpw != 4) x.fpw = 2;
     x.copy_upload = on("NVH_COPY_UPLOAD");
@@ -1019,6 +1020,34 @@
   return nvh_batch_kernels(s ? &s->scratch : nullptr, buf, cap);
 }
 
+extern "C" int nvh_batch_steady_groups(const nvh_batch* b, int* groups) {
+  return nvh_guard([&]() -> int {
+    if (!b || !groups) return NVH_ERR_ARGUMENT;
+    *groups = b->steady_groups;
+    return NVH_OK;
+  });
+}
+
+extern "C" int nvh_stream_steady_groups(const nvh_stream* s, int* groups) {
+  return nvh_batch_steady_groups(s ? &s->scratch : nullptr, groups);
+}
+
+extern "C" int nvh_steady_count(const uint32_t* headers, int frames, int channels, int block1, int* groups) {
+  return nvh_guard([&]() -> int {
+    if (!groups || frames < 0 || (frames > 0 && !headers)) return NVH_ERR_ARGUMENT;
+    *groups = count_steady_groups((const uint8_t*)headers, NVH_SLAB_HDR_WORDS * sizeof(uint32_t), frames, channels, block1);
+    return NVH_OK;
+  });
+}
+
+extern "C" int nvh_stream_pending_steady(const nvh_stream* s, int* groups) {
+  return nvh_guard([&]() -> int {
+    if (!s || !groups) return NVH_ERR_ARGUMENT;
+    if (s->parser->light()) return NVH_ERR_UNSUPPORTED;
+    return pending_steady_groups(s, groups);
+  });
+}
+
 static int batch_out(nvh_batch* b, const nvh_pcm_out* d, void* d_pcm, NamedForm form = kDescriptor) {
   return nvh_guard([&]() -> int {
     nvh_stream* s = b ? b->s : nullptr;
diff --git a/nvorbis_amd/csrc/nvh_format.h b/nvorbis_amd/csrc/nvh_format.h
--- a/nvorbis_amd/csrc/nvh_format.h
+++ b/nvorbis_amd/csrc/nvh_format.h
@@ -144,6 +144,7 @@
 #define NVH_SLAB_GEO(prev_n, next_n, start, valid) \
   ((uint32_t)((prev_n) >> 6) | ((uint32_t)((next_n) >> 6) << 8) | ((uint32_t)((start) >> 6) << 16) | ((uint32_t)((valid) >> 6) << 24))
 #define NVH_SLAB_HDR_VECS 4
+#define NVH_SLAB_HDR_WORDS 16
 #define NVH_SLAB_MAX_CH 8
 #define NVH_SLAB_MAX_COUPLE 4
 struct NvhSlabHdr {
@@ -162,3 +163,27 @@
   uint32_t coupling;
   uint32_t chan[NVH_SLAB_MAX_CH];
 };
+
+#ifdef __HIPCC__
+#define NVH_HD __host__ __device__ inline __attribute__((always_inline))
+#else
+#define NVH_HD inline
+#endif
+NVH_HD bool nvh_steady_frame(const uint32_t* h, uint32_t n, uint32_t want) {
+  const uint32_t flags = h[0] >> 24, xm = (h[0] >> 16) & 0xFFu;
+  const uint32_t geo = NVH_SLAB_GEO(n, (want & NVH_SLAB_EMIT_NEXT) ? n : 0u, 0u, n >> 1);
+  bool ok = (h[0] & 0xFFFFu) == n && xm == (3u | NVH_SLABX_DONE);
+  ok = ok && (flags & (NVH_SLAB_FUSE_FLOOR | NVH_SLAB_FLOOR_FAULT | NVH_SLAB_COUPLE_PASS)) == NVH_SLAB_FUSE_FLOOR;
+  ok = ok && ((h[4] >> 16) & 0xFFu) == (2u | NVH_SLAB_RGEOM_DIGITS | (2u << 4)) && (h[4] >> 24) == 8u;
+  ok = ok && (h[1] & 0xFFFFu) != 0u && (h[4] & 0xFFFFu) != 0u;
+  ok = ok && (h[8] & 0xFFu) == 1u && (h[9] & 0xFFu) == 1u;
+  return ok && (flags & (NVH_SLAB_EMIT_SELF | NVH_SLAB_EMIT_NEXT)) == want && h[13] == geo;
+}
+NVH_HD bool nvh_steady_pair(const uint32_t* h0, const uint32_t* h1, int channels, int block1, bool* import) {
+  const uint32_t n = (uint32_t)block1;
+  const bool imp = ((h0[0] >> 24) & NVH_SLAB_EMIT_SELF) != 0u;
+  if (import) *import = imp;
+  if (channels != 2 || (n != 2048u && n != 1024u)) return false;
+  const uint32_t outer0 = imp ? NVH_SLAB_EMIT_SELF : 0u, outer1 = imp ? NVH_SLAB_EMIT_NEXT : 0u;
+  return nvh_steady_frame(h0, n, NVH_SLAB_EMIT_NEXT | outer0) && nvh_steady_frame(h1, n, NVH_SLAB_EMIT_SELF | outer1);
+}
diff --git a/nvorbis_amd/csrc/nvh_internal.h b/nvorbis_amd/csrc/nvh_internal.h
--- a/nvorbis_amd/csrc/nvh_internal.h
+++ b/nvorbis_amd/csrc/nvh_internal.h
@@ -173,6 +173,7 @@
   bool copy_upload;
   int fpw;
   bool no_walk_two;
+  bool no_steady;
   bool no_prefetch;
   bool uncached_planes;
   bool poison_planes;
@@ -188,6 +189,9 @@
   int phase_mask;
 };
 const NvhToggles& nvh_toggles();
+int count_steady_groups(const uint8_t* slabs, size_t stride_bytes, int nframes, int channels, int block1);
+struct nvh_stream;
+int pending_steady_groups(const nvh_stream* s, int* groups);
 #ifdef NVH_DEBUG
 extern void* g_dbg_buf;
 #define NVH_DBG_LAUNCH , (long long*)g_dbg_buf, nvh_toggles().phase_mask
@@ -421,6 +425,7 @@
   const uint4* d_slabs = nullptr;
   int emit_frames = 0;
   bool emit_planar_ok = true;
+  int steady_groups = 0;
   int fpw = 1;
   bool ola_all = false;
   int ola_count = 0;
diff --git a/nvorbis_amd/csrc/nvh_launch.hip b/nvorbis_amd/csrc/nvh_launch.hip
--- a/nvorbis_amd/csrc/nvh_launch.hip
+++ b/nvorbis_amd/csrc/nvh_launch.hip
@@ -307,6 +307,7 @@
   ola_list.clear();
   b->emit_frames = 0;
   b->fpw = 1;
+  b->steady_groups = 0;
   {
     const int ch = s->setup.channels;
     const bool narrow = ch <= 2 && s->setup.block1 <= 2048 && !s->shared->slab_general;
@@ -388,6 +389,39 @@
   }
 }
 
+int count_steady_groups(const uint8_t* slabs, size_t stride_bytes, int nframes, int channels, int block1) {
+  const NvhToggles& T = nvh_toggles();
+  if (T.no_steady || T.no_walk_two) return 0;
+  int groups = 0;
+  for (int f = 0; f + 1 < nframes; f += 2) {
+    uint32_t h[2][NVH_SLAB_HDR_WORDS];
+    std::memcpy(h[0], slabs + (size_t)f * stride_bytes, sizeof h[0]);
+    std::memcpy(h[1], slabs + ((size_t)f + 1) * stride_bytes, sizeof h[1]);
+    groups += nvh_steady_pair(h[0], h[1], channels, block1, nullptr) ? 1 : 0;
+  }
+  return groups;
+}
+
+int pending_steady_groups(const nvh_stream* s, int* groups) {
+  nvh::FrameBatch& P = const_cast<nvh::FrameBatch&>(s->pending);
+  std::vector<uint32_t> saved;
+  for (const NvhFrame& fr : P.frames) saved.push_back(fr.emit_flags);
+  nvh_batch tmp;
+  std::vector<int> ola_list;
+  assign_emission(const_cast<nvh_stream*>(s), &tmp, P, nvh_toggles().fpw, ola_list);
+  *groups = 0;
+  nvh::SlabBatch SB;
+  const int rc = tmp.fpw == 2 ? nvh::build_slabs(s->setup, s->shared->slab, P, SB) : NVH_ERR_UNSUPPORTED;
+  for (size_t f = 0; f < saved.size(); f++) P.frames[f].emit_flags = saved[f];
+  if (rc == NVH_ERR_UNSUPPORTED) return NVH_OK;
+  if (rc != NVH_OK) return rc;
+  const size_t nf = P.frames.size();
+  std::vector<uint32_t> hdrs(nf * NVH_SLAB_HDR_WORDS);
+  for (size_t f = 0; f < nf; f++) std::memcpy(&hdrs[f * NVH_SLAB_HDR_WORDS], &SB.data[SB.first[f]], NVH_SLAB_HDR_WORDS * sizeof(uint32_t));
+  *groups = count_steady_groups((const uint8_t*)hdrs.data(), NVH_SLAB_HDR_WORDS * sizeof(uint32_t), (int)nf, s->setup.channels, s->setup.block1);
+  return NVH_OK;
+}
+
 static const int64_t kZeroChunkSamples = 4096;
 static int64_t zero_chunk_samples() {
   const int kib = nvh_toggles().zero_chunk_kib;
@@ -562,6 +596,7 @@
         std::memcpy(h + o_sl + f * stride * 16, &SB.data[SB.first[f]], v * 16);
         slab_bytes += (int64_t)v * 16;
       }
+      if (b->fpw == 2) b->steady_groups = count_steady_groups(h + o_sl, stride * 16, (int)nf, s->setup.channels, s->setup.block1);
       b->descriptor_bytes = (int64_t)(nf * sizeof(NvhFrame) + P.chans.size() * sizeof(NvhChan)) + slab_bytes;
       hipStream_t st = s->ctx->stream;
       HIP_TRY(hipMemcpyAsync(b->blob.p, h, o_sl + nf * stride * 16, hipMemcpyHostToDevice, st));
@@ -847,7 +882,7 @@
     A.nframes = b->nframes;
     A.prefetch_prev = 0;
     A.xcd_map = 0;
-    A.walk_two = nvh_toggles().no_walk_two ? 0 : 1;
+    A.walk_two = nvh_toggles().no_walk_two ? 0 : (nvh_toggles().no_steady ? 1 : 3);
     const bool wide = slab_wide(s);
     emitted = b->emit_frames > 0 && d_pcm != nullptr && !b->block_only && !T.no_emit && !s->shared->slab_general && planar_emit &&
               (wide || !out.mapped());
diff --git a/nvorbis_amd/native.py b/nvorbis_amd/native.py
--- a/nvorbis_amd/native.py
+++ b/nvorbis_amd/native.py
@@ -185,6 +185,10 @@
     "nvh_batch_stats": (C.c_int, [_vp, _i64p]),
     "nvh_batch_kernels": (C.c_int, [_vp, C.c_char_p, C.c_int]),
     "nvh_stream_kernels": (C.c_int, [_vp, C.c_char_p, C.c_int]),
+    "nvh_batch_steady_groups": (C.c_int, [_vp, _ip]),
+    "nvh_stream_steady_groups": (C.c_int, [_vp, _ip]),
+    "nvh_stream_pending_steady": (C.c_int, [_vp, _ip]),
+    "nvh_steady_count": (C.c_int, [_vp, C.c_int, C.c_int, C.c_int, _ip]),
     "nvh_batch_synth": (C.c_int, [_vp, _vp, C.c_int64]),
     "nvh_batch_synth_pcm": (C.c_int, [_vp, C.c_int, _vp, C.c_int64]),
     "nvh_batch_synth_planar": (C.c_int, [_vp, C.c_int, _vp, C.c_int64]),
diff --git a/nvorbis_amd/reader.py b/nvorbis_amd/reader.py
--- a/nvorbis_amd/reader.py
+++ b/nvorbis_amd/reader.py
@@ -344,6 +344,11 @@
         check(lib().nvh_batch_kernels(self._h, buf, 256), "nvh_batch_kernels")
         return buf.value.decode().split(",")
 
+    def steady_groups(self):
+        n = C.c_int(0)
+        check(lib().nvh_batch_steady_groups(self._h, C.byref(n)), "nvh_batch_steady_groups")
+        return n.value
+
     def synth(self, d_pcm_ptr, capacity, dtype=np.float32, plane_stride=None, mix=None, channel_map=None):
         d, _, _, _ = _pcm_out(dtype, plane_stride is not None, mix, channel_map, self._stream.channels)
         d.extent = int(capacity if plane_stride is None else plane_stride)
@@ -476,6 +481,16 @@
         buf = C.create_string_buffer(256)
         check(lib().nvh_stream_kernels(self._h, buf, 256), "nvh_stream_kernels")
         return buf.value.decode().split(",")
+
+    def steady_groups(self):
+        n = C.c_int(0)
+        check(lib().nvh_stream_steady_groups(self._h, C.byref(n)), "nvh_stream_steady_groups")
+        return n.value
+
+    def pending_steady(self):
+        n = C.c_int(0)
+        check(lib().nvh_stream_pending_steady(self._h, C.byref(n)), "nvh_stream_pending_steady")
+        return n.value
 
     def pending_slabs(self):
         fr, _ = self.pending()
```
